# b4rtaz/distributed-llama

Hardware: NVIDIA B200
Metric: decode tokens/sec (batch-1 sequence, greedy) + prefill TTFT, Llama-3.1-8B q40 (higher is better)
Workload: dtype q40 weights, q80 activations (int8 dp4a), bf16 KV, f32 accum; 1 GPU; model=llama-3.1-8b, global_batch=1, seq_len=84, prompt_len=64, parallelism=tp1, l2_policy=weights per step (4.22 GB/GPU) >> 126 MB L2, no flush needed

## Files before the change

csrc/cuda/engine.cu:

```cuda
#include <algorithm>
#include <cstdlib>
#include <cstring>
#include <vector>

#include "engine_api.h"
#include "kernels.h"

namespace dl {

uint32_t gHiddenAct = 0;

static_assert(kApiMaxRanks == kMaxRanks, "engine_api.h and kernels.h disagree on the rank limit");

struct Buffers {
    int *tokens, *pos;
    float *x, *qkv, *z, *h, *logits;
    float *attnPartial;
    unsigned int *attnCounters;
    int *history;
    int *expertIdx;
    float *expertWeight;
    float *routerLogits;
    unsigned int *routerCounter;
    float *moeScratch;
    unsigned int *moeCounters;
    int *pTokens, *pPos;
    float *px, *pqkv;
    void *pxn, *pzb, *phb;
    float *pAttnPartial;
    unsigned int *pAttnCounters;
    float *argVal;
    int *argIdx;
    unsigned int *argCounter;
};

struct Engine {
    EngineConfig cfg{};
    CommPtrs comm{};
    bool tp = false;
    std::vector<LayerPtrs> layers;
    GlobalPtrs g{};
    Buffers b{};
    std::vector<void *> kCache, vCache;
    std::vector<void *> owned;
    cudaGraphExec_t decodeGraph = nullptr;
    cudaStream_t captureStream = nullptr;
    int lastError = 0;
    uint64_t *trace = nullptr;
    uint32_t traceCap = 0;
    bool traceAllCtas = false;
    MegaLayer *megaLayers = nullptr;
    unsigned int *megaCounter = nullptr;
    uint2 *megaX2 = nullptr;
    uint32_t megaFlags = 0;
    uint2 *megaX = nullptr, *megaQkv = nullptr, *megaZ = nullptr, *megaH = nullptr;
    unsigned int *megaSeq = nullptr;
    unsigned int *abortHost = nullptr, *abortDev = nullptr;
    uint32_t megaInflight = 2;
    uint32_t megaCtas = 0;
    bool useMega = false;
    bool lastDecodeMega = false, megaFallbackWarned = false;
    unsigned long long *rngState = nullptr;
    float *probScratch = nullptr;
    unsigned int *gatherEpoch = nullptr, *gatherBlockCounter = nullptr;
    float **gatherUcDev = nullptr;
    unsigned int **flagUcDev = nullptr;
    uint32_t vocabLimit = 0;
    bool prefillFusedAr = false;
    bool tcAttn = true;
    bool fusedAttn = true, fusedArgmax = true, useTma = true;
};

#define DL_TRY(expr)                    \
    do {                                \
        const int _r = (expr);          \
        if (_r != 0) return _r;         \
    } while (0)

static EmbTable embTable(const Engine &e) {
    EmbTable t{};
    t.rowsPerRank = e.g.embRowsPerRank;
    if (t.rowsPerRank == 0) t.shard[0] = e.g.embedding;
    else for (int r = 0; r < kMaxRanks; r++) t.shard[r] = e.g.embeddingPeers[r];
    return t;
}

constexpr uint32_t kArenaMaxCtas = 256;

static EngineConfig applyLimits(EngineConfig c) {
    if (c.nExperts > 0) c.maxBatch = 1;
    if (c.maxPrefill > 256) c.maxPrefill = 256;
    return c;
}

struct ArenaLayout {
    uint64_t slotsOff, flagsOff, candValOff, gatherOff, prefillSlotsOff, bytes;
};

static ArenaLayout arenaLayout(const EngineConfig &c) {
    auto align = [](uint64_t x) { return (x + 255) / 256 * 256; };
    ArenaLayout a{};
    uint64_t off = 0;
    a.slotsOff = off; off = align(off + 2ull * c.nRanks * c.maxBatch * c.dim * 8);
    a.flagsOff = off; off = align(off + 2ull * c.nRanks * kArenaMaxCtas * 4);
    a.candValOff = off; off = align(off + kMaxRanks * 8);
    a.gatherOff = off; off = align(off + (uint64_t)c.maxBatch * c.vocabFull * 4);
    a.prefillSlotsOff = off; off = align(off + 2ull * c.nRanks * c.maxPrefill * c.dim * 8);
    a.bytes = off;
    return a;
}

static void fillAr(const Engine &e, ArArgs &ar, uint32_t parity) {
    const EngineConfig &c = e.cfg;
    const ArenaLayout L = arenaLayout(c);
    ar.nRanks = c.nRanks; ar.rank = c.rank; ar.parity = parity; ar.maxCtas = kArenaMaxCtas; ar.slotStride = c.maxBatch * c.dim; ar.dim = c.dim;
    ar.slotsMc = e.comm.mcArena ? (uint64_t *)((uint8_t *)e.comm.mcArena + L.slotsOff) : nullptr;
    for (uint32_t r = 0; r < c.nRanks && r < (uint32_t)kMaxRanks; r++) {
        uint8_t *base = (uint8_t *)e.comm.arena[r];
        ar.slots[r] = (uint64_t *)(base + L.slotsOff);
        ar.cand[r] = (uint64_t *)(base + L.candValOff);
    }
}

static uint32_t localVocabLimit(const Engine &e) {
    return (e.vocabLimit && e.vocabLimit < e.cfg.vocab) ? e.vocabLimit : e.cfg.vocab;
}

static int gemvSel(const Engine &e, int pro, int epi, int nb, const GemvArgs &a, int numSms, cudaStream_t stream, bool pdl) {
    if (e.cfg.wType != 0) return gemvDense((int)e.cfg.wType, pro, epi, nb, a, numSms, stream, pdl);
    if (a.ar.nRanks > 1) {
        const int r = gemvQ40Tma(pro, epi, nb, a, numSms, stream, pdl);
        return r == 1 ? -30 : r;
    }
    return e.useTma ? gemvQ40Auto(pro, epi, nb, a, numSms, stream, pdl) : gemvQ40(pro, epi, nb, a, numSms, stream, pdl);
}

static int runMoe(Engine &e, const LayerPtrs &L, float *out, bool fusedAr, uint64_t *trace13, uint64_t *trace2, cudaStream_t stream,
                  bool pdl) {
    const EngineConfig &c = e.cfg;
    if (c.wType != 0) return -34;
    RouterArgs ro{};
    ro.x = e.b.x; ro.normW = L.norm1; ro.gate = L.moeGate; ro.eps = c.eps; ro.dim = c.dim; ro.nExperts = c.nExperts;
    ro.k = c.nActiveExperts; ro.logits = e.b.routerLogits; ro.counter = e.b.routerCounter; ro.expertIdx = e.b.expertIdx;
    ro.expertWeight = e.b.expertWeight;
    DL_TRY(launchMoeRouter(ro, 1, stream, pdl));
    const uint32_t perSlot = c.numSms / c.nActiveExperts > 0 ? c.numSms / c.nActiveExperts : 1;
    GemvArgs a{};
    a.qs = (const uint32_t *)L.w13Qs; a.scales = (const __half *)L.w13Sc; a.d = 2 * c.ffDim; a.n = c.dim;
    a.in = e.b.x; a.inStride = c.dim; a.normW = L.norm1; a.eps = c.eps; a.out = e.b.h; a.outStride = c.ffDim; a.trace = trace13;
    a.moeCtasPerSlot = perSlot; a.kActive = c.nActiveExperts; a.expertIdx = e.b.expertIdx; a.outSlotStride = c.ffDim;
    a.expertQsStride = (uint64_t)2 * c.ffDim * (c.dim / 8); a.expertScaleStride = (uint64_t)2 * c.ffDim * (c.dim / 32);
    a.moeFirstExpert = c.moeFirstExpert; a.moeNumLocal = c.moeNumLocal;
    { const int r = gemvQ40Tma(PRO_RMSNORM_, EPI_SWIGLU_, 1, a, c.numSms, stream, pdl); if (r != 0) return r == 1 ? -31 : r; }
    a = GemvArgs{};
    a.qs = (const uint32_t *)L.w2Qs; a.scales = (const __half *)L.w2Sc; a.d = c.dim; a.n = c.ffDim;
    a.in = e.b.h; a.inStride = c.ffDim; a.inSlotStride = c.ffDim; a.out = out; a.outStride = c.dim; a.trace = trace2;
    a.moeCtasPerSlot = perSlot; a.kActive = c.nActiveExperts; a.expertIdx = e.b.expertIdx; a.expertWeight = e.b.expertWeight;
    a.expertQsStride = (uint64_t)c.dim * (c.ffDim / 8); a.expertScaleStride = (uint64_t)c.dim * (c.ffDim / 32);
    a.moeFirstExpert = c.moeFirstExpert; a.moeNumLocal = c.moeNumLocal; a.moeScratch = e.b.moeScratch; a.moeCounters = e.b.moeCounters;
    if (fusedAr) fillAr(e, a.ar, 1);
    { const int r = gemvQ40Tma(PRO_PLAIN_, EPI_MOE_DOWN_, 1, a, c.numSms, stream, pdl); if (r != 0) return r == 1 ? -32 : r; }
    return 0;
}

static int engineDecodeMega(Engine &e, bool greedyAdvance, cudaStream_t stream) {
    const EngineConfig &c = e.cfg;
    if (!e.megaLayers || c.nExperts > 0 || c.wType != 0) return 1;
    MegaArgs m{};
    m.layers = e.megaLayers; m.nLayers = c.nLayers; m.dim = c.dim; m.nHeads = c.nHeads; m.nKvHeads = c.nKvHeads; m.headDim = c.headDim;
    m.ffDim = c.ffDim; m.vocab = c.vocab; m.vocabFull = c.vocabFull; m.seqLen = c.seqLen; m.nSplits = c.nSplits; m.eps = c.eps;
    m.embedding = embTable(e); m.finalNorm = e.g.finalNorm; m.rope = e.g.rope;
    m.wclsQs = (const uint8_t *)e.g.wclsQs; m.wclsSc = (const uint8_t *)e.g.wclsSc;
    m.tokens = e.b.tokens; m.pos = e.b.pos; m.history = e.b.history;
    m.logits = e.b.logits; m.maxInflight = e.megaInflight;
    m.xW = e.megaX; m.xW2 = e.megaX2; m.flags = e.megaFlags; m.qkvW = e.megaQkv; m.zW = e.megaZ; m.hF = (float *)e.megaH; m.launchSeq = e.megaSeq; m.abortFlag = e.abortDev;
    m.syncNs = (e.tp && e.megaSeq) ? (unsigned long long *)(e.megaSeq + 2) : nullptr;
    m.attnPartial = e.b.attnPartial; m.attnCounters = e.b.attnCounters;
    m.argVal = e.b.argVal; m.argIdx = e.b.argIdx; m.argCounter = e.b.argCounter; m.gridCounter = e.megaCounter;
    m.rowOffsetGlobal = c.rank * c.vocab; m.greedyAdvance = greedyAdvance ? 1u : 0u; m.vocabLimit = e.vocabLimit;
    m.trace = e.trace;
    m.traceCtas = e.traceAllCtas ? c.numSms : 1u;
    m.traceStride = e.traceAllCtas ? (uint32_t)(((size_t)e.traceCap * 4) / c.numSms) : 0u;
    if (e.tp) fillAr(e, m.ar, 0);
    return launchMegaDecode(m, (int)(e.megaCtas ? e.megaCtas : c.numSms), stream);
}

static int engineForward(Engine &e, int nb, int logitsMode, bool greedyAdvance, cudaStream_t stream) {
    const EngineConfig &c = e.cfg;
    const bool pdl = c.usePdl != 0;
    const uint32_t qDim = c.nHeads * c.headDim, kvDim = c.nKvHeads * c.headDim, qkvDim = qDim + 2 * kvDim;
    if (nb < 1 || (uint32_t)nb > c.maxBatch || (nb & (nb - 1))) return -10;
    e.lastDecodeMega = false;
    if (nb == 1 && logitsMode == 1 && e.useMega) {
        const int r = engineDecodeMega(e, greedyAdvance, stream);
        if (r != 1) { e.lastDecodeMega = r == 0; return r; }
        if (!e.megaFallbackWarned) {
            std::fprintf(stderr, "dl_engine: the persistent decode kernel cannot run this configuration (shape, shared memory or co-residency); "
                                 "using the multi-kernel path\n");
            e.megaFallbackWarned = true;
        }
    }
    uint32_t slot = 0;
    auto nextTrace = [&]() -> uint64_t * { uint64_t *t = (e.trace && slot < e.traceCap) ? e.trace + (size_t)slot * 4 : nullptr; slot++; return t; };

    DL_TRY(launchEmbedding(embTable(e), e.b.tokens, e.b.x, c.dim, c.dim, c.vocabFull, nb, stream));
    for (uint32_t l = 0; l < c.nLayers; l++) {
        const LayerPtrs &L = e.layers[l];
        GemvArgs a{};
        a.qs = (const uint32_t *)L.qkvQs; a.scales = (const __half *)L.qkvSc; a.d = qkvDim; a.n = c.dim;
        a.in = e.b.x; a.inStride = c.dim; a.normW = L.norm0; a.eps = c.eps; a.out = e.b.qkv; a.outStride = qkvDim; a.trace = nextTrace();
        DL_TRY(gemvSel(e, PRO_RMSNORM_, EPI_STORE_, nb, a, c.numSms, stream, pdl));
        if (nb == 1 && e.fusedAttn) {
            AttnFusedArgs f{};
            f.qkv = e.b.qkv; f.pos = e.b.pos; f.rope = e.g.rope; f.qNorm = L.qNorm; f.kNorm = L.kNorm; f.eps = c.eps;
            f.kCache = (__nv_bfloat16 *)e.kCache[l]; f.vCache = (__nv_bfloat16 *)e.vCache[l];
            f.nHeads = c.nHeads; f.nKvHeads = c.nKvHeads; f.headDim = c.headDim; f.seqLen = c.seqLen; f.nSplits = c.nSplits;
            f.partial = e.b.attnPartial; f.counters = e.b.attnCounters; f.out = e.b.z; f.trace = nextTrace();
            DL_TRY(launchAttnFused(f, stream, pdl));
        } else {
            RopeKvArgs r{};
            r.qkv = e.b.qkv; r.qkvStride = qkvDim; r.pos = e.b.pos; r.rope = e.g.rope; r.qNorm = L.qNorm; r.kNorm = L.kNorm;
            r.eps = c.eps; r.nHeads = c.nHeads; r.nKvHeads = c.nKvHeads; r.headDim = c.headDim; r.seqLen = c.seqLen;
            r.kCache = (__nv_bfloat16 *)e.kCache[l]; r.vCache = (__nv_bfloat16 *)e.vCache[l];
            DL_TRY(launchRopeKv(r, nb, stream, pdl));
            AttnArgs t{};
            t.qkv = e.b.qkv; t.qkvStride = qkvDim; t.pos = e.b.pos; t.kCache = r.kCache; t.vCache = r.vCache;
            t.nHeads = c.nHeads; t.nKvHeads = c.nKvHeads; t.headDim = c.headDim; t.seqLen = c.seqLen; t.nSplits = c.nSplits;
            t.partial = e.b.attnPartial; t.counters = e.b.attnCounters; t.out = e.b.z; t.outStride = qDim;
            DL_TRY(launchAttnDecode(t, nb, stream, pdl));
        }
        a = GemvArgs{};
        a.qs = (const uint32_t *)L.woQs; a.scales = (const __half *)L.woSc; a.d = c.dim; a.n = qDim;
        a.in = e.b.z; a.inStride = qDim; a.out = e.b.x; a.outStride = c.dim; a.trace = nextTrace();
        if (e.tp) fillAr(e, a.ar, 0);
        DL_TRY(gemvSel(e, PRO_PLAIN_, EPI_RESIDUAL_, nb, a, c.numSms, stream, pdl));
        if (c.nExperts > 0) {
            if (nb != 1) return -13;
            nextTrace();
            uint64_t *t13 = nextTrace(), *t2 = nextTrace();
            DL_TRY(runMoe(e, L, e.b.x, e.tp, t13, t2, stream, pdl));
            continue;
        }
        a = GemvArgs{};
        a.qs = (const uint32_t *)L.w13Qs; a.scales = (const __half *)L.w13Sc; a.d = 2 * c.ffDim; a.n = c.dim;
        a.in = e.b.x; a.inStride = c.dim; a.normW = L.norm1; a.eps = c.eps; a.out = e.b.h; a.outStride = c.ffDim; a.trace = nextTrace();
        DL_TRY(gemvSel(e, PRO_RMSNORM_, EPI_SWIGLU_, nb, a, c.numSms, stream, pdl));
        a = GemvArgs{};
        a.qs = (const uint32_t *)L.w2Qs; a.scales = (const __half *)L.w2Sc; a.d = c.dim; a.n = c.ffDim;
        a.in = e.b.h; a.inStride = c.ffDim; a.out = e.b.x; a.outStride = c.dim; a.trace = nextTrace();
        if (e.tp) fillAr(e, a.ar, 1);
        DL_TRY(gemvSel(e, PRO_PLAIN_, EPI_RESIDUAL_, nb, a, c.numSms, stream, pdl));
    }
    if (logitsMode != 0) {
        GemvArgs a{};
        a.qs = (const uint32_t *)e.g.wclsQs; a.scales = (const __half *)e.g.wclsSc; a.d = c.vocab; a.n = c.dim;
        a.normW = e.g.finalNorm; a.eps = c.eps; a.inStride = c.dim; a.outStride = c.vocab; a.out = e.b.logits; a.trace = nextTrace();
        if (logitsMode == 1) {
            a.in = e.b.x + (size_t)(nb - 1) * c.dim;
            int r = 1;
            if (greedyAdvance && e.fusedArgmax && c.wType == 0) {
                a.argVal = e.b.argVal; a.argIdx = e.b.argIdx; a.argCounter = e.b.argCounter;
                a.tokenOut = e.b.tokens; a.posInOut = e.b.pos; a.history = e.b.history; a.historyCap = c.seqLen;
                a.rowOffsetGlobal = c.rank * c.vocab; a.vocabLimit = e.vocabLimit;
                if (e.tp) fillAr(e, a.ar, 0);
                r = gemvQ40Tma(PRO_RMSNORM_, EPI_ARGMAX_, 1, a, c.numSms, stream, pdl);
                if (r < 0) return r;
            }
            if (r == 1) {
                if (greedyAdvance && e.tp) return -33;
                a.argVal = nullptr; a.argIdx = nullptr; a.argCounter = nullptr; a.tokenOut = nullptr; a.posInOut = nullptr; a.history = nullptr;
                a.ar = ArArgs{};
                DL_TRY(gemvSel(e, PRO_RMSNORM_, EPI_STORE_, 1, a, c.numSms, stream, pdl));
                if (greedyAdvance)
                    DL_TRY(launchArgmaxAdvance(e.b.logits, localVocabLimit(e), e.b.tokens, e.b.pos, e.b.history, c.seqLen, stream, pdl));
            }
        } else {
            a.in = e.b.x;
            DL_TRY(gemvSel(e, PRO_RMSNORM_, EPI_STORE_, nb, a, c.numSms, stream, pdl));
            if (greedyAdvance) {
                if (e.tp) return -33;
                DL_TRY(launchArgmaxAdvance(e.b.logits, localVocabLimit(e), e.b.tokens, e.b.pos, e.b.history, c.seqLen, stream, pdl));
            }
        }
    }
    return 0;
}

static int enginePrefill(Engine &e, uint32_t T, uint32_t p0, int wantLogits, cudaStream_t stream) {
    const EngineConfig &c = e.cfg;
    const GlobalPtrs &g = e.g;
    const Buffers &b = e.b;
    const bool pdl = c.usePdl != 0;
    const uint32_t qDim = c.nHeads * c.headDim, kvDim = c.nKvHeads * c.headDim, qkvDim = qDim + 2 * kvDim;
    if (T < 1 || T > c.maxPrefill) return -11;
    if (c.wType != 0) return -35;
    const bool tp = e.tp;
    ArArgs arP{};
    if (tp) {
        fillAr(e, arP, 0);
        const uint64_t off = arenaLayout(c).prefillSlotsOff;
        arP.slotStride = c.maxPrefill * c.dim;
        for (uint32_t r = 0; r < c.nRanks; r++) arP.slots[r] = (uint64_t *)((uint8_t *)e.comm.arena[r] + off);
        arP.slotsMc = e.comm.mcArena ? (uint64_t *)((uint8_t *)e.comm.mcArena + off) : nullptr;
    }
    DL_TRY(launchEmbedding(embTable(e), b.pTokens, b.px, c.dim, c.dim, c.vocabFull, (int)T, stream));
    for (uint32_t l = 0; l < c.nLayers; l++) {
        const LayerPtrs &L = e.layers[l];
        DL_TRY(launchRmsNormBf16(b.px, c.dim, L.norm0, b.pxn, c.dim, c.dim, c.eps, T, stream, pdl));
        DL_TRY(gemmQ40Tc(GEPI_STORE_F32_, L.qkvQs, L.qkvSc, qkvDim, c.dim, b.pxn, c.dim, T, b.pqkv, qkvDim, c.numSms, stream, pdl));
        RopeKvArgs r{};
        r.qkv = b.pqkv; r.qkvStride = qkvDim; r.pos = b.pPos; r.rope = g.rope; r.qNorm = L.qNorm; r.kNorm = L.kNorm;
        r.eps = c.eps; r.nHeads = c.nHeads; r.nKvHeads = c.nKvHeads; r.headDim = c.headDim; r.seqLen = c.seqLen;
        r.kCache = (__nv_bfloat16 *)e.kCache[l]; r.vCache = (__nv_bfloat16 *)e.vCache[l];
        DL_TRY(launchRopeKv(r, (int)T, stream, pdl));
        int attnRc = 1;
        if (e.tcAttn) {
            AttnPrefillArgs ap{};
            ap.qkv = b.pqkv; ap.qkvStride = qkvDim; ap.T = T; ap.p0 = p0; ap.nHeads = c.nHeads; ap.nKvHeads = c.nKvHeads;
            ap.headDim = c.headDim; ap.seqLen = c.seqLen; ap.kCache = r.kCache; ap.vCache = r.vCache;
            ap.out = (__nv_bfloat16 *)b.pzb; ap.outStride = qDim;
            attnRc = launchAttnPrefillTc(ap, stream, pdl);
            if (attnRc < 0) return attnRc;
        }
        if (attnRc == 1) {
            AttnArgs t{};
            t.qkv = b.pqkv; t.qkvStride = qkvDim; t.pos = b.pPos; t.kCache = r.kCache; t.vCache = r.vCache;
            t.nHeads = c.nHeads; t.nKvHeads = c.nKvHeads; t.headDim = c.headDim; t.seqLen = c.seqLen; t.nSplits = 1;
            t.partial = b.pAttnPartial; t.counters = b.pAttnCounters; t.out = nullptr; t.outStride = qDim; t.outBf16 = (__nv_bfloat16 *)b.pzb;
            DL_TRY(launchAttnDecode(t, (int)T, stream, pdl));
        }
        if (tp && !e.prefillFusedAr) {
            arP.parity = 0;
            DL_TRY(gemmQ40Tc(GEPI_STORE_F32_, L.woQs, L.woSc, c.dim, qDim, b.pzb, qDim, T, b.pqkv, c.dim, c.numSms, stream, pdl));
            DL_TRY(launchArResidual(b.px, b.pqkv, c.dim, T, arP, stream, pdl));
        } else if (tp) { arP.parity = 0; DL_TRY(gemmQ40TcAr(L.woQs, L.woSc, c.dim, qDim, b.pzb, qDim, T, b.px, c.dim, c.numSms, stream, arP)); }
        else DL_TRY(gemmQ40Tc(GEPI_RESIDUAL_, L.woQs, L.woSc, c.dim, qDim, b.pzb, qDim, T, b.px, c.dim, c.numSms, stream, pdl));
        if (c.nExperts > 0) {
            MoePrefillArgs mo{};
            mo.x = b.px; mo.xnScratch = b.pxn; mo.norm = L.norm1; mo.gate = L.moeGate; mo.w13Qs = L.w13Qs; mo.w13Sc = L.w13Sc;
            mo.w2Qs = L.w2Qs; mo.w2Sc = L.w2Sc; mo.T = T; mo.dim = c.dim; mo.ff = c.ffDim; mo.nExperts = c.nExperts; mo.k = c.nActiveExperts;
            mo.firstLocal = c.moeFirstExpert; mo.nLocal = c.moeNumLocal; mo.eps = c.eps; mo.numSms = (int)c.numSms;
            if (tp) { arP.parity = 1; mo.ar = arP; }
            const int mr = moePrefillFfn(mo, stream);
            if (mr != 0) return mr == 1 ? -36 : mr;
            continue;
        }
        DL_TRY(launchRmsNormBf16(b.px, c.dim, L.norm1, b.pxn, c.dim, c.dim, c.eps, T, stream, pdl));
        DL_TRY(gemmQ40Tc(GEPI_SWIGLU_BF16_, L.w13Qs, L.w13Sc, 2 * c.ffDim, c.dim, b.pxn, c.dim, T, b.phb, c.ffDim, c.numSms, stream, pdl));
        if (tp && !e.prefillFusedAr) {
            arP.parity = 1;
            DL_TRY(gemmQ40Tc(GEPI_STORE_F32_, L.w2Qs, L.w2Sc, c.dim, c.ffDim, b.phb, c.ffDim, T, b.pqkv, c.dim, c.numSms, stream, pdl));
            DL_TRY(launchArResidual(b.px, b.pqkv, c.dim, T, arP, stream, pdl));
        } else if (tp) { arP.parity = 1; DL_TRY(gemmQ40TcAr(L.w2Qs, L.w2Sc, c.dim, c.ffDim, b.phb, c.ffDim, T, b.px, c.dim, c.numSms, stream, arP)); }
        else DL_TRY(gemmQ40Tc(GEPI_RESIDUAL_, L.w2Qs, L.w2Sc, c.dim, c.ffDim, b.phb, c.ffDim, T, b.px, c.dim, c.numSms, stream, pdl));
    }
    if (wantLogits) {
        GemvArgs a{};
        a.qs = (const uint32_t *)g.wclsQs; a.scales = (const __half *)g.wclsSc; a.d = c.vocab; a.n = c.dim;
        a.normW = g.finalNorm; a.eps = c.eps; a.inStride = c.dim; a.outStride = c.vocab; a.out = b.logits;
        a.in = b.px + (size_t)(T - 1) * c.dim;
        DL_TRY(gemvSel(e, PRO_RMSNORM_, EPI_STORE_, 1, a, c.numSms, stream, false));
    }
    return 0;
}

static bool allocBuffers(Engine &e) {
    const EngineConfig &c = e.cfg;
    bool ok = true;
    auto zeroed = [&](size_t bytes) -> void * {
        void *p = nullptr;
        if (!ok || bytes == 0) return nullptr;
        if (cudaMalloc(&p, bytes) != cudaSuccess) { ok = false; return nullptr; }
        e.owned.push_back(p);
        ok = cudaMemset(p, 0, bytes) == cudaSuccess;
        return p;
    };
    const size_t mb = c.maxBatch, mp = c.maxPrefill, dim = c.dim, ff = c.ffDim, heads = c.nHeads, hd = c.headDim;
    const size_t kAct = std::max(1u, c.nActiveExperts), qDim = heads * hd, qkvDim = qDim + 2 * (size_t)c.nKvHeads * hd;
    Buffers &b = e.b;
    b.tokens = (int *)zeroed(mb * 4); b.pos = (int *)zeroed(mb * 4);
    b.x = (float *)zeroed(mb * dim * 4); b.qkv = (float *)zeroed(mb * qkvDim * 4); b.z = (float *)zeroed(mb * qDim * 4);
    b.h = (float *)zeroed(std::max(mb, kAct) * ff * 4); b.logits = (float *)zeroed(mb * c.vocab * 4);
    b.attnPartial = (float *)zeroed(mb * heads * c.nSplits * (hd + 2) * 4); b.attnCounters = (unsigned int *)zeroed(mb * heads * 4);
    b.history = (int *)zeroed(((size_t)c.seqLen + 1) * 4);
    b.expertIdx = (int *)zeroed(mb * kAct * 4); b.expertWeight = (float *)zeroed(mb * kAct * 4);
    b.routerLogits = (float *)zeroed(mb * std::max(1u, c.nExperts) * 4); b.routerCounter = (unsigned int *)zeroed(mb * 4);
    b.moeScratch = (float *)zeroed(kAct * dim * 4); b.moeCounters = (unsigned int *)zeroed(256 * 4);
    b.pTokens = (int *)zeroed(mp * 4); b.pPos = (int *)zeroed(mp * 4);
    b.px = (float *)zeroed(mp * dim * 4); b.pqkv = (float *)zeroed(mp * std::max(qkvDim, dim) * 4);
    b.pxn = zeroed(mp * dim * 2); b.pzb = zeroed(mp * qDim * 2); b.phb = zeroed(mp * ff * 2);
    b.pAttnPartial = (float *)zeroed(mp * heads * (hd + 2) * 4); b.pAttnCounters = (unsigned int *)zeroed(mp * heads * 4);
    b.argVal = (float *)zeroed(256 * 4); b.argIdx = (int *)zeroed(256 * 4); b.argCounter = (unsigned int *)zeroed(4 * 4);
    for (uint32_t l = 0; l < c.nLayers; l++) {
        e.kCache.push_back(zeroed((size_t)c.nKvHeads * c.seqLen * hd * 2));
        e.vCache.push_back(zeroed((size_t)c.nKvHeads * c.seqLen * hd * 2));
    }
    return ok && cudaDeviceSynchronize() == cudaSuccess;
}

}

using dl::Engine;

DL_EXPORT void *dl_engine_create(const dl::EngineConfig *cfg) {
    Engine *e = new Engine();
    e->cfg = dl::applyLimits(*cfg);
    dl::gHiddenAct = cfg->hiddenAct;
    e->layers.resize(cfg->nLayers);
    e->fusedAttn = std::getenv("DL_NO_FUSED_ATTN") == nullptr;
    e->fusedArgmax = std::getenv("DL_NO_FUSED_ARGMAX") == nullptr;
    e->useTma = std::getenv("DL_NO_TMA") == nullptr;
    e->tcAttn = std::getenv("DL_NO_TC_ATTN") == nullptr;
    e->prefillFusedAr = std::getenv("DL_PREFILL_FUSED_AR") != nullptr;
    if (e->cfg.numSms == 0) {
        int dev = 0, sms = 0;
        cudaGetDevice(&dev);
        cudaDeviceGetAttribute(&sms, cudaDevAttrMultiProcessorCount, dev);
        e->cfg.numSms = (uint32_t)sms;
    }
    if (e->cfg.nSplits == 0) e->cfg.nSplits = std::max(1u, std::min(32u, 2 * e->cfg.numSms / std::max(1u, e->cfg.nHeads)));
    if (!dl::allocBuffers(*e)) {
        dl_engine_destroy(e);
        return nullptr;
    }
    return e;
}

DL_EXPORT void dl_engine_destroy(void *h) {
    Engine *e = (Engine *)h;
    if (!e) return;
    if (e->decodeGraph) cudaGraphExecDestroy(e->decodeGraph);
    if (e->captureStream) cudaStreamDestroy(e->captureStream);
    if (e->megaLayers) cudaFree(e->megaLayers);
    if (e->megaCounter) cudaFree(e->megaCounter);
    for (void *q : {(void *)e->megaX, (void *)e->megaX2, (void *)e->megaQkv, (void *)e->megaZ, (void *)e->megaH, (void *)e->megaSeq}) if (q) cudaFree(q);
    if (e->abortHost) cudaFreeHost(e->abortHost);
    for (void *p : e->owned) cudaFree(p);
    delete e;
}

DL_EXPORT int dl_engine_set_layer(void *h, uint32_t layer, const dl::LayerPtrs *p) {
    Engine *e = (Engine *)h;
    if (layer >= e->layers.size()) return -1;
    e->layers[layer] = *p;
    return 0;
}

DL_EXPORT int dl_engine_set_globals(void *h, const dl::GlobalPtrs *p) {
    ((Engine *)h)->g = *p;
    return 0;
}

DL_EXPORT int dl_engine_get_config(void *h, dl::EngineConfig *cfg) {
    *cfg = ((Engine *)h)->cfg;
    return 0;
}

DL_EXPORT int dl_engine_buffers(void *h, dl::EngineBuffers *out) {
    const Engine *e = (Engine *)h;
    const dl::Buffers &b = e->b;
    *out = dl::EngineBuffers{b.tokens, b.pos, b.history, b.logits, b.x, b.pTokens, b.pPos, e->kCache.data(), e->vCache.data()};
    return 0;
}

DL_EXPORT size_t dl_engine_arena_bytes(const dl::EngineConfig *cfg) { return dl::arenaLayout(dl::applyLimits(*cfg)).bytes; }

DL_EXPORT int dl_engine_enable_mega(void *h, int enable) {
    Engine *e = (Engine *)h;
    if (enable && !e->megaLayers) {
        std::vector<dl::MegaLayer> tab(e->layers.size());
        for (size_t l = 0; l < tab.size(); l++) {
            const dl::LayerPtrs &L = e->layers[l];
            dl::MegaLayer &m = tab[l];
            m.qkvQs = (const uint8_t *)L.qkvQs; m.qkvSc = (const uint8_t *)L.qkvSc; m.woQs = (const uint8_t *)L.woQs; m.woSc = (const uint8_t *)L.woSc;
            m.w13Qs = (const uint8_t *)L.w13Qs; m.w13Sc = (const uint8_t *)L.w13Sc; m.w2Qs = (const uint8_t *)L.w2Qs; m.w2Sc = (const uint8_t *)L.w2Sc;
            m.norm0 = L.norm0; m.norm1 = L.norm1; m.qNorm = L.qNorm; m.kNorm = L.kNorm;
            m.kCache = (__nv_bfloat16 *)e->kCache[l]; m.vCache = (__nv_bfloat16 *)e->vCache[l];
        }
        DL_CUDA_CHECK(cudaMalloc(&e->megaLayers, tab.size() * sizeof(dl::MegaLayer)));
        DL_CUDA_CHECK(cudaMemcpy(e->megaLayers, tab.data(), tab.size() * sizeof(dl::MegaLayer), cudaMemcpyHostToDevice));
        DL_CUDA_CHECK(cudaMalloc(&e->megaCounter, 256));
        DL_CUDA_CHECK(cudaMemset(e->megaCounter, 0, 256));
        const dl::EngineConfig &c = e->cfg;
        const size_t qDim = (size_t)c.nHeads * c.headDim, qkvDim = qDim + 2 * (size_t)c.nKvHeads * c.headDim;
        auto allocW = [](uint2 **p, size_t n) {
            const size_t bytes = (n + 8) * sizeof(uint2);
            if (cudaMalloc(p, bytes) != cudaSuccess) return false;
            return cudaMemset(*p, 0, bytes) == cudaSuccess;
        };
        if (!allocW(&e->megaX, c.dim) || !allocW(&e->megaX2, c.dim) || !allocW(&e->megaQkv, qkvDim) || !allocW(&e->megaZ, qDim) || !allocW(&e->megaH, c.ffDim)) return -41;
        DL_CUDA_CHECK(cudaMalloc(&e->megaSeq, 256));
        const unsigned int one = 1;
        DL_CUDA_CHECK(cudaMemset(e->megaSeq, 0, 256));
        DL_CUDA_CHECK(cudaMemcpy(e->megaSeq, &one, sizeof(one), cudaMemcpyHostToDevice));
        if (!e->abortHost) {
            DL_CUDA_CHECK(cudaHostAlloc((void **)&e->abortHost, 64, cudaHostAllocMapped));
            std::memset(e->abortHost, 0, 64);
            DL_CUDA_CHECK(cudaHostGetDevicePointer((void **)&e->abortDev, e->abortHost, 0));
        }
        if (const char *g = std::getenv("DL_MEGA_CTAS")) e->megaCtas = (uint32_t)std::atoi(g);
        if (const char *g = std::getenv("DL_MEGA_FLAGS")) e->megaFlags = (uint32_t)std::atoi(g);
        if (const char *g = std::getenv("DL_MEGA_INFLIGHT")) e->megaInflight = (uint32_t)std::atoi(g);
    }
    e->useMega = enable != 0;
    return 0;
}

DL_EXPORT int dl_engine_set_vocab_limit(void *h, uint32_t limit) {
    Engine *e = (Engine *)h;
    if (e->vocabLimit != limit && e->decodeGraph) { cudaGraphExecDestroy(e->decodeGraph); e->decodeGraph = nullptr; }
    e->vocabLimit = limit;
    return 0;
}

DL_EXPORT unsigned long long dl_engine_sync_ns(void *h) {
    Engine *e = (Engine *)h;
    unsigned long long v = 0;
    if (e->megaSeq && cudaMemcpy(&v, e->megaSeq + 2, sizeof(v), cudaMemcpyDeviceToHost) != cudaSuccess) return 0ull;
    return v;
}

DL_EXPORT int dl_engine_aborted(void *h) {
    Engine *e = (Engine *)h;
    return (e->abortHost && *e->abortHost) ? 1 : 0;
}

DL_EXPORT int dl_engine_sampler_seed(void *h, unsigned long long seed) {
    Engine *e = (Engine *)h;
    const dl::EngineConfig &c = e->cfg;
    if (!e->rngState) {
        DL_CUDA_CHECK(cudaMalloc(&e->rngState, 64));
        DL_CUDA_CHECK(cudaMalloc(&e->probScratch, ((size_t)c.vocab * (c.nRanks ? c.nRanks : 1) + 16) * sizeof(float)));
        DL_CUDA_CHECK(cudaMalloc(&e->gatherEpoch, 64));
        DL_CUDA_CHECK(cudaMemset(e->gatherEpoch, 0, 64));
        DL_CUDA_CHECK(cudaMalloc(&e->gatherBlockCounter, 64));
        DL_CUDA_CHECK(cudaMemset(e->gatherBlockCounter, 0, 64));
        if (e->tp) {
            const dl::ArenaLayout L = dl::arenaLayout(c);
            float *g[dl::kApiMaxRanks] = {};
            unsigned int *f[dl::kApiMaxRanks] = {};
            for (uint32_t r = 0; r < c.nRanks; r++) {
                g[r] = (float *)((uint8_t *)e->comm.arena[r] + L.gatherOff);
                f[r] = (unsigned int *)((uint8_t *)e->comm.arena[r] + L.flagsOff);
            }
            DL_CUDA_CHECK(cudaMalloc(&e->gatherUcDev, sizeof(g)));
            DL_CUDA_CHECK(cudaMalloc(&e->flagUcDev, sizeof(f)));
            DL_CUDA_CHECK(cudaMemcpy(e->gatherUcDev, g, sizeof(g), cudaMemcpyHostToDevice));
            DL_CUDA_CHECK(cudaMemcpy(e->flagUcDev, f, sizeof(f), cudaMemcpyHostToDevice));
        }
    }
    if (seed == 0) seed = 0x9E3779B97F4A7C15ull;
    DL_CUDA_CHECK(cudaMemcpy(e->rngState, &seed, sizeof(seed), cudaMemcpyHostToDevice));
    return 0;
}

DL_EXPORT int dl_engine_sample(void *h, float temperature, float topp, cudaStream_t stream) {
    Engine *e = (Engine *)h;
    const dl::EngineConfig &c = e->cfg;
    if (!e->rngState) return -50;
    const uint32_t nR = e->tp ? c.nRanks : 1;
    const uint32_t full = c.vocab * nR;
    const uint32_t n = (e->vocabLimit && e->vocabLimit < full) ? e->vocabLimit : full;
    if (nR == 1)
        return dl::launchSample(e->b.logits, e->probScratch, n, temperature, topp, e->rngState, e->b.tokens, e->b.pos, e->b.history, c.seqLen,
                                nullptr, nullptr, 1, stream);
    const dl::ArenaLayout L = dl::arenaLayout(c);
    uint8_t *mine = (uint8_t *)e->comm.arena[c.rank];
    float *gatherLocal = (float *)(mine + L.gatherOff);
    unsigned int *flagLocal = (unsigned int *)(mine + L.flagsOff);
    float *gatherMc = e->comm.mcArena ? (float *)((uint8_t *)e->comm.mcArena + L.gatherOff) : nullptr;
    unsigned int *flagMc = e->comm.mcArena ? (unsigned int *)((uint8_t *)e->comm.mcArena + L.flagsOff) : nullptr;
    DL_TRY(dl::launchLogitsGather(e->b.logits, c.vocab, c.rank, nR, gatherMc, e->gatherUcDev, flagMc, e->flagUcDev, e->gatherBlockCounter, stream));
    return dl::launchSample(gatherLocal, e->probScratch, n, temperature, topp, e->rngState, e->b.tokens, e->b.pos, e->b.history, c.seqLen, flagLocal,
                            e->gatherEpoch, nR, stream);
}

DL_EXPORT int dl_engine_set_comm(void *h, const dl::CommPtrs *p) {
    Engine *e = (Engine *)h;
    e->comm = *p;
    e->tp = e->cfg.nRanks > 1;
    return 0;
}

DL_EXPORT int dl_engine_set_trace(void *h, uint64_t *buf, uint32_t capLaunches) {
    ((Engine *)h)->trace = buf;
    ((Engine *)h)->traceCap = capLaunches;
    return 0;
}

DL_EXPORT int dl_engine_set_trace_all(void *h, int allCtas) {
    ((Engine *)h)->traceAllCtas = allCtas != 0;
    return 0;
}

DL_EXPORT int dl_engine_mega_active(void *h) { return ((Engine *)h)->lastDecodeMega ? 1 : 0; }

DL_EXPORT int dl_engine_forward(void *h, int nb, int logitsMode, int greedyAdvance, cudaStream_t stream) {
    return dl::engineForward(*(Engine *)h, nb, logitsMode, greedyAdvance != 0, stream);
}

DL_EXPORT int dl_engine_forward_part(void *h, int nb, uint32_t layer, int part, float *ybuf, cudaStream_t stream) {
    Engine &e = *(Engine *)h;
    const dl::EngineConfig &c = e.cfg;
    const uint32_t qDim = c.nHeads * c.headDim, kvDim = c.nKvHeads * c.headDim, qkvDim = qDim + 2 * kvDim;
    if (nb < 1 || (uint32_t)nb > c.maxBatch || (nb & (nb - 1))) return -10;
    if (part == 0) return dl::launchEmbedding(embTable(e), e.b.tokens, e.b.x, c.dim, c.dim, c.vocabFull, nb, stream);
    if (part == 3 || part == 4) {
        dl::GemvArgs a{};
        a.qs = (const uint32_t *)e.g.wclsQs; a.scales = (const __half *)e.g.wclsSc; a.d = c.vocab; a.n = c.dim;
        a.normW = e.g.finalNorm; a.eps = c.eps; a.inStride = c.dim; a.outStride = c.vocab; a.out = e.b.logits;
        a.in = part == 3 ? e.b.x + (size_t)(nb - 1) * c.dim : e.b.x;
        return dl::gemvSel(e, dl::PRO_RMSNORM_, dl::EPI_STORE_, part == 3 ? 1 : nb, a, c.numSms, stream, false);
    }
    if (layer >= c.nLayers) return -1;
    const dl::LayerPtrs &L = e.layers[layer];
    dl::GemvArgs a{};
    if (part == 1) {
        a.qs = (const uint32_t *)L.qkvQs; a.scales = (const __half *)L.qkvSc; a.d = qkvDim; a.n = c.dim;
        a.in = e.b.x; a.inStride = c.dim; a.normW = L.norm0; a.eps = c.eps; a.out = e.b.qkv; a.outStride = qkvDim;
        DL_TRY(dl::gemvSel(e, dl::PRO_RMSNORM_, dl::EPI_STORE_, nb, a, c.numSms, stream, false));
        dl::RopeKvArgs r{};
        r.qkv = e.b.qkv; r.qkvStride = qkvDim; r.pos = e.b.pos; r.rope = e.g.rope; r.qNorm = L.qNorm; r.kNorm = L.kNorm;
        r.eps = c.eps; r.nHeads = c.nHeads; r.nKvHeads = c.nKvHeads; r.headDim = c.headDim; r.seqLen = c.seqLen;
        r.kCache = (__nv_bfloat16 *)e.kCache[layer]; r.vCache = (__nv_bfloat16 *)e.vCache[layer];
        DL_TRY(dl::launchRopeKv(r, nb, stream, false));
        dl::AttnArgs t{};
        t.qkv = e.b.qkv; t.qkvStride = qkvDim; t.pos = e.b.pos; t.kCache = r.kCache; t.vCache = r.vCache;
        t.nHeads = c.nHeads; t.nKvHeads = c.nKvHeads; t.headDim = c.headDim; t.seqLen = c.seqLen; t.nSplits = c.nSplits;
        t.partial = e.b.attnPartial; t.counters = e.b.attnCounters; t.out = e.b.z; t.outStride = qDim;
        DL_TRY(dl::launchAttnDecode(t, nb, stream, false));
        a = dl::GemvArgs{};
        a.qs = (const uint32_t *)L.woQs; a.scales = (const __half *)L.woSc; a.d = c.dim; a.n = qDim;
        a.in = e.b.z; a.inStride = qDim; a.out = ybuf; a.outStride = c.dim;
        return dl::gemvSel(e, dl::PRO_PLAIN_, dl::EPI_STORE_, nb, a, c.numSms, stream, false);
    }
    if (part == 2 && c.nExperts > 0) {
        if (nb != 1) return -13;
        DL_CUDA_CHECK(cudaMemsetAsync(ybuf, 0, (size_t)c.dim * sizeof(float), stream));
        return dl::runMoe(e, L, ybuf, false, nullptr, nullptr, stream, false);
    }
    if (part == 2) {
        a.qs = (const uint32_t *)L.w13Qs; a.scales = (const __half *)L.w13Sc; a.d = 2 * c.ffDim; a.n = c.dim;
        a.in = e.b.x; a.inStride = c.dim; a.normW = L.norm1; a.eps = c.eps; a.out = e.b.h; a.outStride = c.ffDim;
        DL_TRY(dl::gemvSel(e, dl::PRO_RMSNORM_, dl::EPI_SWIGLU_, nb, a, c.numSms, stream, false));
        a = dl::GemvArgs{};
        a.qs = (const uint32_t *)L.w2Qs; a.scales = (const __half *)L.w2Sc; a.d = c.dim; a.n = c.ffDim;
        a.in = e.b.h; a.inStride = c.ffDim; a.out = ybuf; a.outStride = c.dim;
        return dl::gemvSel(e, dl::PRO_PLAIN_, dl::EPI_STORE_, nb, a, c.numSms, stream, false);
    }
    return -2;
}

DL_EXPORT int dl_engine_prefill(void *h, uint32_t T, uint32_t p0, int wantLogits, cudaStream_t stream) {
    return dl::enginePrefill(*(Engine *)h, T, p0, wantLogits, stream);
}

DL_EXPORT int dl_engine_capture_decode(void *h) {
    Engine *e = (Engine *)h;
    if (!e->captureStream) DL_CUDA_CHECK(cudaStreamCreateWithFlags(&e->captureStream, cudaStreamNonBlocking));
    if (e->decodeGraph) { cudaGraphExecDestroy(e->decodeGraph); e->decodeGraph = nullptr; }
    DL_CUDA_CHECK(cudaStreamBeginCapture(e->captureStream, cudaStreamCaptureModeThreadLocal));
    const int r = dl::engineForward(*e, 1, 1, true, e->captureStream);
    cudaGraph_t graph = nullptr;
    const cudaError_t endErr = cudaStreamEndCapture(e->captureStream, &graph);
    if (r != 0) { if (graph) cudaGraphDestroy(graph); return r; }
    DL_CUDA_CHECK(endErr);
    DL_CUDA_CHECK(cudaGraphInstantiate(&e->decodeGraph, graph, 0));
    cudaGraphDestroy(graph);
    return 0;
}

DL_EXPORT int dl_engine_decode_graph(void *h, int nSteps, cudaStream_t stream) {
    Engine *e = (Engine *)h;
    if (!e->decodeGraph) return -20;
    for (int i = 0; i < nSteps; i++) DL_CUDA_CHECK(cudaGraphLaunch(e->decodeGraph, stream));
    return 0;
}
```

csrc/cuda/kernels.h:

```cpp
#pragma once
#include "common.cuh"

namespace dl {

enum { PRO_RMSNORM_ = 0, PRO_PLAIN_ = 1 };
enum { EPI_STORE_ = 0, EPI_RESIDUAL_ = 1, EPI_SWIGLU_ = 2, EPI_ARGMAX_ = 3, EPI_MOE_DOWN_ = 4 };

constexpr int kMaxRanks = 8;
extern uint32_t gHiddenAct;

struct ArArgs {
    uint32_t nRanks, rank, parity, maxCtas;
    uint32_t slotStride;
    uint32_t dim;
    uint64_t *slots[kMaxRanks];
    uint64_t *cand[kMaxRanks];
    uint64_t *slotsMc;
};

struct GemvArgs {
    const uint32_t *qs;
    const __half *scales;
    uint32_t d, n;
    const float *in;
    const float *normW;
    float eps;
    float *out;
    uint32_t inStride, outStride;
    uint32_t maxTileRows;
    const int *expertIdx;
    uint32_t slot, kActive;
    uint64_t expertQsStride, expertScaleStride;
    const float *expertWeight;
    float *argVal;
    int *argIdx;
    unsigned int *argCounter;
    int *tokenOut, *posInOut, *history;
    uint32_t historyCap;
    uint32_t rowOffsetGlobal;
    uint64_t *trace;
    uint32_t moeCtasPerSlot, moeFirstExpert, moeNumLocal;
    uint32_t inSlotStride, outSlotStride;
    float *moeScratch;
    unsigned int *moeCounters;
    ArArgs ar;
    uint32_t act;
    uint32_t vocabLimit;
};
int gemvQ40(int pro, int epi, int nb, GemvArgs a, int numSms, cudaStream_t stream, bool pdl);
int gemvQ40Tma(int pro, int epi, int nb, GemvArgs a, int numSms, cudaStream_t stream, bool pdl);
inline int gemvQ40Auto(int pro, int epi, int nb, const GemvArgs &a, int numSms, cudaStream_t stream, bool pdl) {
    const int r = gemvQ40Tma(pro, epi, nb, a, numSms, stream, pdl);
    return r == 1 ? gemvQ40(pro, epi, nb, a, numSms, stream, pdl) : r;
}

int gemvDense(int wtype, int pro, int epi, int nb, GemvArgs a, int numSms, cudaStream_t stream, bool pdl);

struct RopeKvArgs {
    float *qkv;
    uint32_t qkvStride;
    const int *pos;
    const float *rope;
    const float *qNorm;
    const float *kNorm;
    float eps;
    uint32_t nHeads, nKvHeads, headDim, seqLen;
    __nv_bfloat16 *kCache;
    __nv_bfloat16 *vCache;
};
int launchRopeKv(const RopeKvArgs &a, int nb, cudaStream_t stream, bool pdl);

struct AttnArgs {
    const float *qkv;
    uint32_t qkvStride;
    const int *pos;
    const __nv_bfloat16 *kCache, *vCache;
    uint32_t nHeads, nKvHeads, headDim, seqLen, nSplits;
    float *partial;
    unsigned int *counters;
    float *out;
    uint32_t outStride;
    __nv_bfloat16 *outBf16;
};
int launchAttnDecode(const AttnArgs &a, int nb, cudaStream_t stream, bool pdl);

struct AttnPrefillArgs {
    const float *qkv;
    uint32_t qkvStride;
    uint32_t T, p0;
    uint32_t nHeads, nKvHeads, headDim, seqLen;
    const __nv_bfloat16 *kCache, *vCache;
    __nv_bfloat16 *out;
    uint32_t outStride;
};
int launchAttnPrefillTc(const AttnPrefillArgs &a, cudaStream_t stream, bool pdl = false);

struct AttnFusedArgs {
    const float *qkv;
    const int *pos;
    const float *rope;
    const float *qNorm, *kNorm;
    float eps;
    __nv_bfloat16 *kCache, *vCache;
    uint32_t nHeads, nKvHeads, headDim, seqLen, nSplits;
    float *partial;
    unsigned int *counters;
    float *out;
    uint64_t *trace;
};
int launchAttnFused(const AttnFusedArgs &a, cudaStream_t stream, bool pdl);

struct RouterArgs {
    const float *x;
    const float *normW;
    const float *gate;
    float eps;
    uint32_t dim, nExperts, k;
    float *logits;
    unsigned int *counter;
    int *expertIdx;
    float *expertWeight;
};
int launchMoeRouter(const RouterArgs &a, int nb, cudaStream_t stream, bool pdl);

struct EmbTable {
    const float *shard[kMaxRanks];
    uint32_t rowsPerRank;
    __host__ __device__ const float *row(uint32_t tok, uint32_t dim) const {
        if (rowsPerRank == 0) return shard[0] + (size_t)tok * dim;
        const uint32_t r = tok / rowsPerRank;
        return shard[r] + (size_t)(tok - r * rowsPerRank) * dim;
    }
};
int launchEmbedding(const EmbTable &table, const int *tokens, float *x, uint32_t dim, uint32_t xStride, uint32_t vocab, int nb,
                    cudaStream_t stream);
int launchArgmaxAdvance(const float *logits, uint32_t vocab, int *tokenOut, int *pos, int *history, uint32_t historyCap,
                        cudaStream_t stream, bool pdl);

int launchSample(const float *logits, float *probs, uint32_t n, float temperature, float topp, unsigned long long *rng, int *tokenOut, int *pos,
                 int *history, uint32_t historyCap, const unsigned int *gatherFlag, unsigned int *gatherEpoch, uint32_t nRanks,
                 cudaStream_t stream);
int launchLogitsGather(const float *local, uint32_t v0, uint32_t rank, uint32_t nRanks, float *gatherMc, float *const *gatherUcDev,
                       unsigned int *flagMc, unsigned int *const *flagUcDev, unsigned int *blockCounter, cudaStream_t stream);

struct MegaLayer {
    const uint8_t *qkvQs, *qkvSc, *woQs, *woSc, *w13Qs, *w13Sc, *w2Qs, *w2Sc;
    const float *norm0, *norm1, *qNorm, *kNorm;
    __nv_bfloat16 *kCache, *vCache;
};

struct MegaPhase {
    uint32_t d, n, nblk, nseg;
    uint32_t stageRows;
    uint32_t pairsQ, pairsRem;
    uint32_t recipNseg, gInc, segInc, rotInc;
};

struct MegaArgs {
    const MegaLayer *layers;
    uint32_t nLayers, dim, nHeads, nKvHeads, headDim, ffDim, vocab, vocabFull, seqLen, nSplits;
    float eps;
    EmbTable embedding;
    const float *finalNorm, *rope;
    const uint8_t *wclsQs, *wclsSc;
    int *tokens, *pos, *history;
    float *logits;
    uint2 *xW2;
    uint32_t flags;
    uint2 *xW, *qkvW, *zW;
    float *hF;
    unsigned int *launchSeq;
    unsigned int *abortFlag;
    unsigned long long *syncNs;
    float *attnPartial;
    unsigned int *attnCounters;
    float *argVal;
    int *argIdx;
    unsigned int *argCounter;
    unsigned int *gridCounter;
    uint32_t stageBytes, nStages, planeBlocks, partialFloats;
    uint32_t maxInflight;
    MegaPhase ph[5];
    uint32_t rowOffsetGlobal;
    uint32_t greedyAdvance;
    uint32_t act, vocabLimit;
    uint64_t *trace;
    uint32_t traceCtas, traceStride;
    ArArgs ar;
};

int launchMegaDecode(MegaArgs m, int numSms, cudaStream_t stream);

enum { GEPI_STORE_F32_ = 0, GEPI_RESIDUAL_ = 1, GEPI_SWIGLU_BF16_ = 2, GEPI_STORE_BF16_ = 3 };
int gemmQ40Tc(int epi, const void *qs, const void *scales, uint32_t d, uint32_t n, const void *act, uint32_t actStride, uint32_t T,
              void *out, uint32_t outStride, int numSms, cudaStream_t stream, bool pdl);
int gemmQ40TcAr(const void *qs, const void *scales, uint32_t d, uint32_t n, const void *act, uint32_t actStride, uint32_t T, void *out,
                uint32_t outStride, int numSms, cudaStream_t stream, const ArArgs &ar);
int gemmQ40TcGrouped(int epi, const void *qs, const void *scales, uint32_t nGroups, uint32_t grpRows, uint32_t n, const void *act,
                     uint32_t actStride, uint32_t rowsTotal, uint32_t maxTokens, const int *grpCount, const int *grpOffset, void *out,
                     uint32_t outStride, int numSms, cudaStream_t stream);
struct MoePrefillArgs {
    float *x;
    void *xnScratch;
    const float *norm, *gate;
    const void *w13Qs, *w13Sc, *w2Qs, *w2Sc;
    uint32_t T, dim, ff, nExperts, k, firstLocal, nLocal;
    float eps;
    int numSms;
    ArArgs ar;
};
int moePrefillFfn(const MoePrefillArgs &a, cudaStream_t stream);
template <typename... KArgs, typename... Args>
inline cudaError_t launchPdl(void (*kernel)(KArgs...), dim3 grid, dim3 block, size_t smem, cudaStream_t stream, bool pdl, Args... args) {
    cudaLaunchConfig_t cfg{};
    cfg.gridDim = grid; cfg.blockDim = block; cfg.dynamicSmemBytes = smem; cfg.stream = stream;
    cudaLaunchAttribute attr[1];
    attr[0].id = cudaLaunchAttributeProgrammaticStreamSerialization;
    attr[0].val.programmaticStreamSerializationAllowed = pdl ? 1 : 0;
    cfg.attrs = attr; cfg.numAttrs = 1;
    return cudaLaunchKernelEx(&cfg, kernel, KArgs(args)...);
}

int launchArResidual(float *x, const float *partial, uint32_t dim, uint32_t T, const ArArgs &ar, cudaStream_t stream, bool pdl = false);
int launchRmsNormBf16(const float *x, uint32_t xStride, const float *w, void *y, uint32_t yStride, uint32_t n, float eps, uint32_t T,
                      cudaStream_t stream, bool pdl = false);

}
```

csrc/cuda/mega_decode.cu:

```cuda
#include <type_traits>

#include "kernels.h"
#include "tma_common.cuh"

namespace dl {

enum { MP_QKV = 0, MP_WO = 1, MP_W13 = 2, MP_W2 = 3, MP_LOGITS = 4 };

static uint32_t megaStageRows(uint32_t n, uint32_t stageBytes) {
    const uint32_t rowBytes = (n / 32) * 18;
    uint32_t sr = stageBytes / rowBytes;
    sr = sr / 4 * 4;
    return sr > 64 ? 64 : sr;
}

struct MegaSmem {
    uint8_t *ring;
    uint4 *planeA, *planeB;
    float *dxs, *dx8, *partial, *red, *rope;
    uint64_t *fullBar, *emptyBar;
};

constexpr uint32_t kSpinCheck = 1u << 12;
constexpr uint32_t kSpinLimit = 1u << 27;

struct SpinGuard {
    volatile unsigned int *abortFlag;
    uint32_t n = 0;
    __device__ __forceinline__ explicit SpinGuard(unsigned int *f) : abortFlag(f) {}
    __device__ __forceinline__ bool tick() {
        if ((++n & (kSpinCheck - 1)) != 0) return false;
        if (abortFlag && *abortFlag) return true;
        if (n >= kSpinLimit) {
            if (abortFlag) *abortFlag = 1u;
            return true;
        }
        return false;
    }
};

__device__ __forceinline__ void gridBarrier(unsigned int *ctr, unsigned int &target, int tid, unsigned int *abortFlag) {
    consumerBarrier();
    if (tid == 0) {
        asm volatile("red.relaxed.gpu.global.add.u32 [%0], 1;" ::"l"(ctr) : "memory");
        target += gridDim.x;
        unsigned int v;
        SpinGuard g(abortFlag);
        do {
            asm volatile("ld.relaxed.gpu.global.u32 %0, [%1];" : "=r"(v) : "l"(ctr) : "memory");
        } while (v < target && !g.tick());
    }
    consumerBarrier();
}

__device__ __forceinline__ void gridBarrierFenced(unsigned int *ctr, unsigned int &target, int tid, unsigned int *abortFlag) {
    consumerBarrier();
    if (tid == 0) {
        asm volatile("red.release.gpu.global.add.u32 [%0], 1;" ::"l"(ctr) : "memory");
        target += gridDim.x;
        unsigned int v;
        SpinGuard g(abortFlag);
        do {
            asm volatile("ld.acquire.gpu.global.u32 %0, [%1];" : "=r"(v) : "l"(ctr) : "memory");
        } while (v < target && !g.tick());
    }
    consumerBarrier();
}

__device__ __forceinline__ void stW(uint2 *p, float v, uint32_t epoch) {
    asm volatile("st.relaxed.gpu.global.v2.u32 [%0], {%1, %2};" ::"l"(p), "r"(__float_as_uint(v)), "r"(epoch) : "memory");
}
__device__ __forceinline__ uint4 ldW2(const uint2 *p) {
    uint4 v;
    asm volatile("ld.relaxed.gpu.global.v4.u32 {%0, %1, %2, %3}, [%4];" : "=r"(v.x), "=r"(v.y), "=r"(v.z), "=r"(v.w) : "l"(p) : "memory");
    return v;
}
__device__ __forceinline__ uint2 ldW(const uint2 *p) {
    uint2 v;
    asm volatile("ld.relaxed.gpu.global.v2.u32 {%0, %1}, [%2];" : "=r"(v.x), "=r"(v.y) : "l"(p) : "memory");
    return v;
}
__device__ __forceinline__ float ldWwait(const uint2 *p, uint32_t epoch, unsigned int *abortFlag) {
    uint2 v = ldW(p);
    if (v.y != epoch) {
        SpinGuard g(abortFlag);
        do { __nanosleep(100); v = ldW(p); } while (v.y != epoch && !g.tick());
    }
    return __uint_as_float(v.x);
}
__device__ __forceinline__ float4 ldW4wait(const uint2 *base, uint32_t i4, uint32_t epoch, unsigned int *abortFlag) {
    const uint2 *p = base + (size_t)i4 * 4;
    uint4 a = ldW2(p), b = ldW2(p + 2);
    if (a.y != epoch || a.w != epoch || b.y != epoch || b.w != epoch) {
        SpinGuard g(abortFlag);
        do { __nanosleep(100); a = ldW2(p); b = ldW2(p + 2); } while ((a.y != epoch || a.w != epoch || b.y != epoch || b.w != epoch) && !g.tick());
    }
    return make_float4(__uint_as_float(a.x), __uint_as_float(a.z), __uint_as_float(b.x), __uint_as_float(b.z));
}

struct RingPos {
    uint32_t st, par;
    __device__ __forceinline__ void advance(uint32_t nStages) {
        if (++st == nStages) { st = 0; par ^= 1u; }
    }
};

__device__ __forceinline__ void megaTile(const MegaPhase &P, uint32_t &pairBegin, uint32_t &tileRows) {
    const uint32_t b = blockIdx.x;
    pairBegin = b * P.pairsQ + min(b, P.pairsRem);
    tileRows = 2 * (P.pairsQ + (b < P.pairsRem ? 1u : 0u));
}

template <int PRO, int EPI, bool IN_PLAIN = false>
__device__ void megaGemv(const MegaArgs &m, const MegaSmem &sm, const MegaPhase &P, const uint2 *in, uint32_t inEpoch, const float *normW,
                         uint2 *outW, uint32_t outEpoch, float *outF, uint32_t arParity, RingPos &ring, int tid, uint32_t &slot,
                         const float *inF = nullptr, const uint2 *resW = nullptr) {
    auto stamp = [&]() { if (m.trace && tid == 0 && blockIdx.x < m.traceCtas) m.trace[(size_t)blockIdx.x * m.traceStride + slot] = globalTimerNs(); slot++; };
    const int lane = tid & 31, warp = tid >> 5;
    const uint32_t n = P.n;
    const uint32_t nblk = P.nblk, nseg = P.nseg;
    const uint32_t rowQsBytes = nblk * 16;
    uint32_t pairBegin, tileRows;
    megaTile(P, pairBegin, tileRows);
    const uint32_t rowBase = pairBegin * 2;
    const uint32_t SR = P.stageRows;
    uint4 *planeA = sm.planeA, *planeB = sm.planeB;
    float *dxs = sm.dxs, *dx8 = sm.dx8, *partial = sm.partial, *red = sm.red;

    float resid = 0.f;
    if (EPI == EPI_RESIDUAL_ && (uint32_t)tid < tileRows) resid = __uint_as_float(ldW((resW ? resW : outW) + rowBase + tid).x);

    {
        const uint32_t nVec = n / 4;
        constexpr int kMaxVec = PRO == PRO_RMSNORM_ ? 4 : 8;
        constexpr uint32_t kChunkVec = kMaxVec * kConsumerThreads;
        uint8_t *pa = reinterpret_cast<uint8_t *>(planeA);
        uint8_t *pb = reinterpret_cast<uint8_t *>(planeB);
        for (uint32_t vecBase = 0; vecBase < nVec; vecBase += kChunkVec) {
            float4 xv[kMaxVec];
            float4 wv[PRO == PRO_RMSNORM_ ? kMaxVec : 1];
            if (PRO == PRO_RMSNORM_) {
#pragma unroll
                for (int k = 0; k < kMaxVec; k++) {
                    const uint32_t i = vecBase + k * kConsumerThreads + tid;
                    wv[k] = i < nVec ? __ldg(reinterpret_cast<const float4 *>(normW) + i) : make_float4(0.f, 0.f, 0.f, 0.f);
                }
            }
            float ss = 0.f;
#pragma unroll
            for (int k = 0; k < kMaxVec; k++) {
                const uint32_t i = vecBase + k * kConsumerThreads + tid;
                if (IN_PLAIN) xv[k] = i < nVec ? __ldcg(reinterpret_cast<const float4 *>(inF) + i) : make_float4(0.f, 0.f, 0.f, 0.f);
                else xv[k] = i < nVec ? ldW4wait(in, i, inEpoch, m.abortFlag) : make_float4(0.f, 0.f, 0.f, 0.f);
                ss += xv[k].x * xv[k].x + xv[k].y * xv[k].y + xv[k].z * xv[k].z + xv[k].w * xv[k].w;
            }
            float inv = 1.f;
            if (PRO == PRO_RMSNORM_) {
                ss = consumerSum(ss, red);
                inv = rsqrtf(ss / (float)n + m.eps);
            }
#pragma unroll
            for (int k = 0; k < kMaxVec; k++) {
                const uint32_t i = vecBase + k * kConsumerThreads + tid;
                if (vecBase + k * kConsumerThreads >= nVec) break;
                const bool act = i < nVec;
                float4 v = xv[k];
                if (PRO == PRO_RMSNORM_ && act) {
                    const float4 w = wv[PRO == PRO_RMSNORM_ ? k : 0];
                    v.x = w.x * (v.x * inv); v.y = w.y * (v.y * inv); v.z = w.z * (v.z * inv); v.w = w.w * (v.w * inv);
                }
                float amax = fmaxf(fmaxf(fabsf(v.x), fabsf(v.y)), fmaxf(fabsf(v.z), fabsf(v.w)));
                amax = fmaxf(amax, __shfl_xor_sync(0xffffffffu, amax, 1));
                amax = fmaxf(amax, __shfl_xor_sync(0xffffffffu, amax, 2));
                amax = fmaxf(amax, __shfl_xor_sync(0xffffffffu, amax, 4));
                const float dq = amax / 127.f;
                const float id = dq != 0.f ? 1.f / dq : 0.f;
                const int q0 = __float2int_rn(v.x * id), q1 = __float2int_rn(v.y * id);
                const int q2 = __float2int_rn(v.z * id), q3 = __float2int_rn(v.w * id);
                int qsum = q0 + q1 + q2 + q3;
                qsum += __shfl_xor_sync(0xffffffffu, qsum, 1);
                qsum += __shfl_xor_sync(0xffffffffu, qsum, 2);
                qsum += __shfl_xor_sync(0xffffffffu, qsum, 4);
                if (act) {
                    const uint32_t b = i >> 3, sub = i & 7, kk = sub >> 1, odd = sub & 1;
                    uint8_t *wa = pa + (size_t)b * 16 + kk * 4 + odd;
                    uint8_t *wb = pb + (size_t)b * 16 + kk * 4 + odd;
                    wa[0] = (uint8_t)(int8_t)q0; wa[2] = (uint8_t)(int8_t)q1;
                    wb[0] = (uint8_t)(int8_t)q2; wb[2] = (uint8_t)(int8_t)q3;
                    if (sub == 0) {
                        const float dr = __half2float(__float2half_rn(dq));
                        dxs[b] = dr;
                        dx8[b] = dr * 8.f * (float)qsum;
                    }
                }
            }
        }
    }
    consumerBarrier();
    stamp();

    const uint32_t gInc = P.gInc, segInc = P.segInc;
    uint32_t rot = 0;
    for (uint32_t r0 = 0; r0 < tileRows; r0 += SR) {
        const uint32_t st = ring.st;
        const uint32_t rows = min(SR, tileRows - r0);
        const uint32_t nSteps = ((rows + kRowsPerStep - 1) / kRowsPerStep) * nseg;
        const uint8_t *stage = sm.ring + st * m.stageBytes;
        const uint4 *sq = reinterpret_cast<const uint4 *>(stage);
        const uint16_t *ss = reinterpret_cast<const uint16_t *>(stage + SR * rowQsBytes);
        const uint32_t firstStep = ((uint32_t)warp - rot) & (kConsumerWarps - 1);
        rot = (rot + P.rotInc) & (kConsumerWarps - 1);
        uint32_t g = (firstStep * P.recipNseg) >> 16, seg = firstStep - g * nseg;
        mbarWait(&sm.fullBar[st], ring.par);
        auto stepDot = [&](uint32_t g_, uint32_t seg_, float (&acc)[kRowsPerStep]) {
            const uint32_t blk = seg_ * 32 + lane;
            const uint32_t rl = g_ * kRowsPerStep;
#pragma unroll
            for (int r = 0; r < kRowsPerStep; r++) acc[r] = 0.f;
            if (blk < nblk) {
                const uint4 A = planeA[blk], B = planeB[blk];
                const float dxv = dxs[blk], dx8v = dx8[blk];
                const uint4 *qp = sq + rl * nblk + blk;
                const uint16_t *sp = ss + rl * nblk + blk;
#pragma unroll
                for (int r = 0; r < kRowsPerStep; r++) {
                    const uint4 q = qp[r * nblk];
                    const float dw = __half2float(__ushort_as_half(sp[r * nblk]));
                    const uint32_t ml = 0x0f0f0f0fu, mh = 0xf0f0f0f0u;
                    int lo = dp4a(q.x & ml, A.x, 0), hi = dp4a(q.x & mh, B.x, 0);
                    lo = dp4a(q.y & ml, A.y, lo); hi = dp4a(q.y & mh, B.y, hi);
                    lo = dp4a(q.z & ml, A.z, lo); hi = dp4a(q.z & mh, B.z, hi);
                    lo = dp4a(q.w & ml, A.w, lo); hi = dp4a(q.w & mh, B.w, hi);
                    acc[r] = dw * (dxv * (float)(lo + (hi >> 4)) - dx8v);
                }
            }
        };
        auto stepStore = [&](uint32_t g_, uint32_t seg_, float v) {
            const uint32_t rl = g_ * kRowsPerStep;
            if ((lane & 7) == 0) {
                const uint32_t r = lane >> 3;
                if (rl + r < rows) partial[(r0 + rl + r) * nseg + seg_] = v;
            }
        };
        auto advance = [&](uint32_t &g_, uint32_t &seg_) {
            g_ += gInc;
            seg_ += segInc;
            if (seg_ >= nseg) { seg_ -= nseg; g_++; }
        };
        uint32_t s = firstStep;
        for (; s + kConsumerWarps < nSteps; s += 2 * kConsumerWarps) {
            uint32_t g2 = g, seg2 = seg;
            advance(g2, seg2);
            float a0[kRowsPerStep], a1[kRowsPerStep];
            stepDot(g, seg, a0);
            stepDot(g2, seg2, a1);
            const float v0 = reduce4(a0[0], a0[1], a0[2], a0[3], lane);
            const float v1 = reduce4(a1[0], a1[1], a1[2], a1[3], lane);
            stepStore(g, seg, v0);
            stepStore(g2, seg2, v1);
            g = g2; seg = seg2;
            advance(g, seg);
        }
        if (s < nSteps) {
            float a0[kRowsPerStep];
            stepDot(g, seg, a0);
            stepStore(g, seg, reduce4(a0[0], a0[1], a0[2], a0[3], lane));
        }
        __syncwarp();
        if (lane == 0) mbarArrive(&sm.emptyBar[st]);
        ring.advance(m.nStages);
    }
    consumerBarrier();
    stamp();

    auto rowSum = [&](uint32_t r) {
        float v = 0.f;
        for (uint32_t sg = 0; sg < nseg; sg++) v += partial[r * nseg + sg];
        return v;
    };
    if (EPI == EPI_SWIGLU_) {
        for (uint32_t p = tid; p < tileRows / 2; p += kConsumerThreads) outF[pairBegin + p] = gateAct(rowSum(2 * p), m.act) * rowSum(2 * p + 1);
    } else if (EPI == EPI_STORE_) {
        for (uint32_t r = tid; r < tileRows; r += kConsumerThreads) stW(outW + rowBase + r, rowSum(r), outEpoch);
    } else if (EPI == EPI_RESIDUAL_) {
        if (m.ar.nRanks > 1) {
            const ArArgs &ar = m.ar;
            const size_t slotBase = (size_t)(arParity * ar.nRanks + ar.rank) * ar.slotStride;
            if ((uint32_t)tid < tileRows) {
                const uint32_t r = tid;
                const float v = rowSum(r);
                if (ar.slotsMc) {
                    const uint64_t word = (uint64_t)__float_as_uint(v) | (1ull << 32);
                    asm volatile("multimem.st.relaxed.sys.global.b64 [%0], %1;" ::"l"(ar.slotsMc + slotBase + rowBase + r), "l"(word) : "memory");
                } else {
#pragma unroll 1
                    for (uint32_t p = 0; p < ar.nRanks; p++) stLL(ar.slots[(ar.rank + p) % ar.nRanks] + slotBase + rowBase + r, __float_as_uint(v), 1u);
                }
                uint64_t *mine = ar.slots[ar.rank];
                float sum = 0.f;
                SpinGuard g(m.abortFlag);
                const bool timeIt = m.syncNs && blockIdx.x == 0 && tid == 0;
                const uint64_t tSync0 = timeIt ? globalTimerNs() : 0;
                for (uint32_t sr = 0; sr < ar.nRanks; sr++) {
                    uint64_t *w = mine + (size_t)(arParity * ar.nRanks + sr) * ar.slotStride + rowBase + r;
                    uint2 v2 = ldLL(w);
                    while (v2.y == 0u && !g.tick()) v2 = ldLL(w);
                    sum += __uint_as_float(v2.x);
                    stLL(w, 0u, 0u);
                }
                if (timeIt) *m.syncNs += globalTimerNs() - tSync0;
                stW(outW + rowBase + r, resid + sum, outEpoch);
            }
        } else if ((uint32_t)tid < tileRows) {
            stW(outW + rowBase + tid, resid + rowSum(tid), outEpoch);
        }
    } else {
        float best = -INFINITY;
        int bestIdx = 0x7fffffff;
        for (uint32_t r = tid; r < tileRows; r += kConsumerThreads) {
            const float v = rowSum(r);
            outF[rowBase + r] = v;
            if (EPI == EPI_ARGMAX_ && v > best && m.rowOffsetGlobal + rowBase + r < m.vocabLimit) { best = v; bestIdx = (int)(m.rowOffsetGlobal + rowBase + r); }
        }
        if (EPI == EPI_ARGMAX_) {
            auto better = [](float v, int i, float bv, int bi) { return v > bv || (v == bv && i < bi); };
#pragma unroll
            for (int o = 16; o > 0; o >>= 1) {
                const float ov = __shfl_xor_sync(0xffffffffu, best, o);
                const int oi = __shfl_xor_sync(0xffffffffu, bestIdx, o);
                if (better(ov, oi, best, bestIdx)) { best = ov; bestIdx = oi; }
            }
            float *sv = red;
            int *si = reinterpret_cast<int *>(red + 16);
            consumerBarrier();
            if (lane == 0) { sv[warp] = best; si[warp] = bestIdx; }
            consumerBarrier();
            __shared__ bool lastCta;
            if (warp == 0) {
                best = lane < kConsumerWarps ? sv[lane] : -INFINITY;
                bestIdx = lane < kConsumerWarps ? si[lane] : 0x7fffffff;
#pragma unroll
                for (int o = 16; o > 0; o >>= 1) {
                    const float ov = __shfl_xor_sync(0xffffffffu, best, o);
                    const int oi = __shfl_xor_sync(0xffffffffu, bestIdx, o);
                    if (better(ov, oi, best, bestIdx)) { best = ov; bestIdx = oi; }
                }
                if (lane == 0) {
                    m.argVal[blockIdx.x] = best;
                    m.argIdx[blockIdx.x] = bestIdx;
                    __threadfence();
                    const unsigned int prev = atomicAdd(m.argCounter, 1u);
                    lastCta = prev == gridDim.x - 1;
                    if (lastCta) *m.argCounter = 0;
                }
            }
            consumerBarrier();
            if (lastCta && warp == 0) {
                __threadfence();
                best = -INFINITY;
                bestIdx = 0x7fffffff;
                for (uint32_t i = lane; i < gridDim.x; i += 32) {
                    const float v = __ldcg(m.argVal + i);
                    const int ix = __ldcg(m.argIdx + i);
                    if (better(v, ix, best, bestIdx)) { best = v; bestIdx = ix; }
                }
#pragma unroll
                for (int o = 16; o > 0; o >>= 1) {
                    const float ov = __shfl_xor_sync(0xffffffffu, best, o);
                    const int oi = __shfl_xor_sync(0xffffffffu, bestIdx, o);
                    if (better(ov, oi, best, bestIdx)) { best = ov; bestIdx = oi; }
                }
                if (m.ar.nRanks > 1) {
                    const ArArgs &ar = m.ar;
                    if (lane < ar.nRanks) stLL(ar.cand[lane] + ar.rank, __float_as_uint(best), (uint32_t)bestIdx + 1u);
                    if (lane < ar.nRanks) {
                        uint64_t *w = ar.cand[ar.rank] + lane;
                        uint2 v = ldLL(w);
                        SpinGuard g(m.abortFlag);
                        while (v.y == 0u && !g.tick()) v = ldLL(w);
                        best = __uint_as_float(v.x);
                        bestIdx = (int)(v.y - 1u);
                        stLL(w, 0u, 0u);
                    } else {
                        best = -INFINITY;
                        bestIdx = 0x7fffffff;
                    }
#pragma unroll
                    for (int o = 16; o > 0; o >>= 1) {
                        const float ov = __shfl_xor_sync(0xffffffffu, best, o);
                        const int oi = __shfl_xor_sync(0xffffffffu, bestIdx, o);
                        if (better(ov, oi, best, bestIdx)) { best = ov; bestIdx = oi; }
                    }
                }
                if (lane == 0 && m.greedyAdvance) {
                    m.tokens[0] = bestIdx;
                    const int p = m.pos[0] + 1;
                    m.pos[0] = p;
                    if (m.history && (uint32_t)p < m.seqLen) m.history[p] = bestIdx;
                }
            }
        }
    }
}

template <int HD>
__device__ void megaAttention(const MegaArgs &m, const MegaSmem &sm, const MegaLayer &L, int p, int tid, uint32_t inEpoch, uint32_t outEpoch) {
    constexpr int DPL = HD / 32;
    const int lane = tid & 31, warp = tid >> 5;
    const uint32_t nPos = (uint32_t)p + 1;
    uint32_t eff = (nPos + 255) / 256;
    if (eff > m.nSplits) eff = m.nSplits;
    if (eff < 1) eff = 1;
    const uint32_t kvMul = m.nHeads / m.nKvHeads;
    const uint32_t qDim = m.nHeads * HD, kvDim = m.nKvHeads * HD;
    float *sAcc = sm.partial;
    float *sM = sm.partial + 16 * HD;
    float *sL = sM + 16;
    __shared__ bool sLast;
    const float2 *ropeRow = reinterpret_cast<const float2 *>(sm.rope) + lane * (DPL / 2);
    auto normRope = [&](float *v, const float *nw) {
        if (nw) {
            float ss = 0.f;
#pragma unroll
            for (int i = 0; i < DPL; i++) ss += v[i] * v[i];
            ss = warpSum(ss);
            const float inv = rsqrtf(ss / (float)HD + m.eps);
#pragma unroll
            for (int i = 0; i < DPL; i++) v[i] = nw[lane * DPL + i] * (v[i] * inv);
        }
#pragma unroll
        for (int k = 0; k < DPL / 2; k++) {
            const float2 cs = ropeRow[k];
            const float x0 = v[2 * k] * cs.x - v[2 * k + 1] * cs.y;
            const float x1 = v[2 * k] * cs.y + v[2 * k + 1] * cs.x;
            v[2 * k] = x0; v[2 * k + 1] = x1;
        }
    };
    for (uint32_t item = blockIdx.x; item < m.nHeads * eff; item += gridDim.x) {
        const uint32_t h = item / eff, split = item - h * eff;
        const uint32_t kvh = h / kvMul;
        const uint32_t chunk = (nPos + eff - 1) / eff;
        const uint32_t begin = split * chunk;
        const uint32_t end = min(begin + chunk, nPos);
        const bool ownsNew = end == nPos;
        const uint32_t cachedEnd = ownsNew ? end - 1 : end;
        __nv_bfloat16 *kHead = L.kCache + (size_t)kvh * m.seqLen * HD;
        __nv_bfloat16 *vHead = L.vCache + (size_t)kvh * m.seqLen * HD;
        const __nv_bfloat16 *kBase = kHead + lane * DPL;
        const __nv_bfloat16 *vBase = vHead + lane * DPL;
        constexpr int UN = 4;
        using RawT = typename std::conditional<DPL == 4, uint2, uint32_t>::type;
        RawT kRaw[UN], vRaw[UN];
        auto loadBatch = [&](uint32_t s0) {
#pragma unroll
            for (int u = 0; u < UN; u++) {
                const uint32_t s = s0 + u;
                if (s < cachedEnd) {
                    kRaw[u] = *reinterpret_cast<const RawT *>(kBase + (size_t)s * HD);
                    vRaw[u] = *reinterpret_cast<const RawT *>(vBase + (size_t)s * HD);
                }
            }
        };
        auto unpack = [&](const RawT &r, float (&o)[DPL]) {
            if constexpr (DPL == 4) {
                const float2 a0 = __bfloat1622float2(*reinterpret_cast<const __nv_bfloat162 *>(&r.x));
                const float2 a1 = __bfloat1622float2(*reinterpret_cast<const __nv_bfloat162 *>(&r.y));
                o[0] = a0.x; o[1] = a0.y; o[2] = a1.x; o[3] = a1.y;
            } else {
                const float2 a0 = __bfloat1622float2(*reinterpret_cast<const __nv_bfloat162 *>(&r));
                o[0] = a0.x; o[1] = a0.y;
            }
        };
        uint32_t s0 = begin + warp * UN;
        loadBatch(s0);
        const bool newRow = ownsNew && warp == 0;
        const uint2 *ksrc = m.qkvW + qDim + (size_t)kvh * HD + lane * DPL;
        const uint2 *vsrc = m.qkvW + qDim + kvDim + (size_t)kvh * HD + lane * DPL;
        float q[DPL], kn[DPL], vn[DPL];
        {
            const uint2 *src = m.qkvW + (size_t)h * HD + lane * DPL;
            if constexpr (DPL == 4) {
                uint4 ka0, ka1, va0, va1;
                if (newRow) { ka0 = ldW2(ksrc); ka1 = ldW2(ksrc + 2); va0 = ldW2(vsrc); va1 = ldW2(vsrc + 2); }
                const float4 v = ldW4wait(src, 0, inEpoch, m.abortFlag);
                q[0] = v.x; q[1] = v.y; q[2] = v.z; q[3] = v.w;
                if (newRow) {
                    if (ka0.y != inEpoch || ka0.w != inEpoch || ka1.y != inEpoch || ka1.w != inEpoch || va0.y != inEpoch || va0.w != inEpoch ||
                        va1.y != inEpoch || va1.w != inEpoch) {
                        const float4 a = ldW4wait(ksrc, 0, inEpoch, m.abortFlag), bq = ldW4wait(vsrc, 0, inEpoch, m.abortFlag);
                        kn[0] = a.x; kn[1] = a.y; kn[2] = a.z; kn[3] = a.w;
                        vn[0] = bq.x; vn[1] = bq.y; vn[2] = bq.z; vn[3] = bq.w;
                    } else {
                        kn[0] = __uint_as_float(ka0.x); kn[1] = __uint_as_float(ka0.z); kn[2] = __uint_as_float(ka1.x); kn[3] = __uint_as_float(ka1.z);
                        vn[0] = __uint_as_float(va0.x); vn[1] = __uint_as_float(va0.z); vn[2] = __uint_as_float(va1.x); vn[3] = __uint_as_float(va1.z);
                    }
                }
            } else {
#pragma unroll
                for (int i = 0; i < DPL; i++) q[i] = ldWwait(src + i, inEpoch, m.abortFlag);
                if (newRow) {
#pragma unroll
                    for (int i = 0; i < DPL; i++) { kn[i] = ldWwait(ksrc + i, inEpoch, m.abortFlag); vn[i] = ldWwait(vsrc + i, inEpoch, m.abortFlag); }
                }
            }
        }
        normRope(q, L.qNorm);
        const float scale = rsqrtf((float)HD);
#pragma unroll
        for (int i = 0; i < DPL; i++) q[i] *= scale;
        float mx = -INFINITY, l = 0.f, acc[DPL];
#pragma unroll
        for (int i = 0; i < DPL; i++) acc[i] = 0.f;
        if (newRow) {
            normRope(kn, L.kNorm);
            __nv_bfloat162 kb[DPL / 2], vb[DPL / 2];
#pragma unroll
            for (int k = 0; k < DPL / 2; k++) {
                kb[k] = __floats2bfloat162_rn(kn[2 * k], kn[2 * k + 1]);
                vb[k] = __floats2bfloat162_rn(vn[2 * k], vn[2 * k + 1]);
                const float2 kf = __bfloat1622float2(kb[k]), vf = __bfloat1622float2(vb[k]);
                kn[2 * k] = kf.x; kn[2 * k + 1] = kf.y;
                vn[2 * k] = vf.x; vn[2 * k + 1] = vf.y;
            }
            if (h % kvMul == 0) {
                __nv_bfloat162 *kd = reinterpret_cast<__nv_bfloat162 *>(kHead + (size_t)p * HD + lane * DPL);
                __nv_bfloat162 *vd = reinterpret_cast<__nv_bfloat162 *>(vHead + (size_t)p * HD + lane * DPL);
#pragma unroll
                for (int k = 0; k < DPL / 2; k++) { kd[k] = kb[k]; vd[k] = vb[k]; }
            }
            float dsum = 0.f;
#pragma unroll
            for (int i = 0; i < DPL; i++) dsum += q[i] * kn[i];
            dsum = warpSum(dsum);
            mx = dsum; l = 1.f;
#pragma unroll
            for (int i = 0; i < DPL; i++) acc[i] = vn[i];
        }
        for (; s0 < cachedEnd; s0 += kConsumerWarps * UN) {
            float kf[UN][DPL], vf[UN][DPL];
#pragma unroll
            for (int u = 0; u < UN; u++) {
                if (s0 + u < cachedEnd) { unpack(kRaw[u], kf[u]); unpack(vRaw[u], vf[u]); }
                else {
#pragma unroll
                    for (int i = 0; i < DPL; i++) { kf[u][i] = 0.f; vf[u][i] = 0.f; }
                }
            }
            const uint32_t cur = s0;
            if (s0 + kConsumerWarps * UN < cachedEnd) loadBatch(s0 + kConsumerWarps * UN);
            float sc[UN];
#pragma unroll
            for (int u = 0; u < UN; u++) {
                float dsum = 0.f;
#pragma unroll
                for (int i = 0; i < DPL; i++) dsum += q[i] * kf[u][i];
                sc[u] = warpSum(dsum);
            }
#pragma unroll
            for (int u = 0; u < UN; u++) {
                if (cur + u < cachedEnd) {
                    const float mNew = fmaxf(mx, sc[u]);
                    const float corr = __expf(mx - mNew);
                    const float pr = __expf(sc[u] - mNew);
                    l = l * corr + pr;
#pragma unroll
                    for (int i = 0; i < DPL; i++) acc[i] = acc[i] * corr + pr * vf[u][i];
                    mx = mNew;
                }
            }
        }
        consumerBarrier();
#pragma unroll
        for (int i = 0; i < DPL; i++) sAcc[warp * HD + lane * DPL + i] = acc[i];
        if (lane == 0) { sM[warp] = mx; sL[warp] = l; }
        consumerBarrier();
        float M = -INFINITY;
#pragma unroll
        for (int w = 0; w < kConsumerWarps; w++) M = fmaxf(M, sM[w]);
        float num = 0.f, Lsum = 0.f;
        if (tid < HD) {
#pragma unroll
            for (int w = 0; w < kConsumerWarps; w++) {
                const float wgt = (sM[w] == -INFINITY) ? 0.f : __expf(sM[w] - M);
                num += sAcc[w * HD + tid] * wgt;
                Lsum += sL[w] * wgt;
            }
        }
        uint2 *outRow = m.zW + (size_t)h * HD;
        if (eff == 1) {
            if (tid < HD) stW(outRow + tid, num / Lsum, outEpoch);
            continue;
        }
        float *pOut = m.attnPartial + ((size_t)h * m.nSplits + split) * (HD + 2);
        if (tid < HD) pOut[tid] = num;
        if (tid == 0) { pOut[HD] = M; pOut[HD + 1] = Lsum; }
        __threadfence();
        consumerBarrier();
        if (tid == 0) {
            const unsigned int prev = atomicAdd(&m.attnCounters[h], 1u);
            sLast = (prev == eff - 1);
            if (sLast) m.attnCounters[h] = 0;
        }
        consumerBarrier();
        if (sLast) {
            __threadfence();
            const float *pIn = m.attnPartial + (size_t)h * m.nSplits * (HD + 2);
            float gM = -INFINITY;
            for (uint32_t s = 0; s < eff; s++) gM = fmaxf(gM, __ldcg(pIn + (size_t)s * (HD + 2) + HD));
            if (tid < HD) {
                float n2 = 0.f, den = 0.f;
                for (uint32_t s = 0; s < eff; s++) {
                    const float w = __expf(__ldcg(pIn + (size_t)s * (HD + 2) + HD) - gM);
                    n2 += w * __ldcg(pIn + (size_t)s * (HD + 2) + tid);
                    den += w * __ldcg(pIn + (size_t)s * (HD + 2) + HD + 1);
                }
                stW(outRow + tid, n2 / den, outEpoch);
            }
        }
    }
}

template <int HD>
__global__ void __launch_bounds__(kTmaThreads, 1) megaDecodeKernel(const __grid_constant__ MegaArgs m) {
    extern __shared__ __align__(128) uint8_t smem[];
    const int tid = threadIdx.x, lane = tid & 31, warp = tid >> 5;
    MegaSmem sm;
    sm.ring = smem;
    sm.planeA = reinterpret_cast<uint4 *>(smem + (size_t)m.nStages * m.stageBytes);
    sm.planeB = sm.planeA + m.planeBlocks;
    sm.dxs = reinterpret_cast<float *>(sm.planeB + m.planeBlocks);
    sm.dx8 = sm.dxs + m.planeBlocks;
    sm.partial = sm.dx8 + m.planeBlocks;
    sm.red = sm.partial + m.partialFloats;
    sm.rope = sm.red + 32;
    sm.fullBar = reinterpret_cast<uint64_t *>(sm.rope + 128);
    sm.emptyBar = sm.fullBar + kMaxStages;

    if (tid == 0) {
        for (uint32_t s = 0; s < m.nStages; s++) {
            mbarInit(&sm.fullBar[s], 1);
            mbarInit(&sm.emptyBar[s], kConsumerWarps);
        }
        asm volatile("fence.mbarrier_init.release.cluster;" ::: "memory");
    }
    __syncthreads();
    const uint32_t qDim = m.nHeads * m.headDim, kvDim = m.nKvHeads * m.headDim, qkvDim = qDim + 2 * kvDim;

    if (warp == kConsumerWarps) {
        if (lane == 0) {
            const uint64_t policy = policyEvictFirst();
            RingPos pr{0u, 0u};
            bool wrapped = false;
            RingPos landed{0u, 0u};
            uint32_t nIssued = 0, nLanded = 0;
            const uint32_t maxInflight = m.maxInflight ? m.maxInflight : m.nStages;
            auto stream = [&](const uint8_t *qs, const uint8_t *sc, const MegaPhase &P) {
                const uint32_t rowQsBytes = P.nblk * 16, rowScBytes = P.nblk * 2;
                uint32_t pairBegin, tileRows;
                megaTile(P, pairBegin, tileRows);
                const uint32_t rowBase = pairBegin * 2, SR = P.stageRows;
                for (uint32_t r0 = 0; r0 < tileRows; r0 += SR) {
                    const uint32_t st = pr.st;
                    if (wrapped) mbarWait(&sm.emptyBar[st], pr.par ^ 1u);
                    while (nIssued - nLanded >= maxInflight) {
                        mbarWait(&sm.fullBar[landed.st], landed.par);
                        landed.advance(m.nStages);
                        nLanded++;
                    }
                    nIssued++;
                    const uint32_t rows = min(SR, tileRows - r0);
                    const uint32_t bq = rows * rowQsBytes, bs = rows * rowScBytes;
                    uint8_t *dst = sm.ring + st * m.stageBytes;
                    mbarExpectTx(&sm.fullBar[st], bq + bs);
                    tmaBulkLoad(dst, qs + (uint64_t)(rowBase + r0) * rowQsBytes, bq, &sm.fullBar[st], policy);
                    tmaBulkLoad(dst + SR * rowQsBytes, sc + (uint64_t)(rowBase + r0) * rowScBytes, bs, &sm.fullBar[st], policy);
                    pr.advance(m.nStages);
                    if (pr.st == 0) wrapped = true;
                }
            };
            for (uint32_t l = 0; l < m.nLayers; l++) {
                const MegaLayer &L = m.layers[l];
                stream(L.qkvQs, L.qkvSc, m.ph[MP_QKV]);
                stream(L.woQs, L.woSc, m.ph[MP_WO]);
                stream(L.w13Qs, L.w13Sc, m.ph[MP_W13]);
                stream(L.w2Qs, L.w2Sc, m.ph[MP_W2]);
            }
            stream(m.wclsQs, m.wclsSc, m.ph[MP_LOGITS]);
        }
        return;
    }

    unsigned int barTarget = 0;
    RingPos ring{0u, 0u};
    uint32_t slot = 0;
    auto stamp = [&]() { if (m.trace && tid == 0 && blockIdx.x < m.traceCtas) m.trace[(size_t)blockIdx.x * m.traceStride + slot] = globalTimerNs(); slot++; };
    stamp();
    const uint32_t seqBase = __ldcg(m.launchSeq) << 10;
    int p = m.pos[0];
    if (p < 0) p = 0;
    if ((uint32_t)p >= m.seqLen) p = m.seqLen - 1;
    if (tid < HD) sm.rope[tid] = m.rope[(size_t)p * HD + tid];
    {
        int tok = m.tokens[0];
        if (tok < 0 || (uint32_t)tok >= m.vocabFull) tok = 0;
        uint32_t pairBegin, tileRows;
        megaTile(m.ph[MP_WO], pairBegin, tileRows);
        if ((uint32_t)tid < tileRows) stW(m.xW + pairBegin * 2 + tid, m.embedding.row((uint32_t)tok, m.dim)[pairBegin * 2 + tid], seqBase);
    }
    gridBarrier(m.gridCounter, barTarget, tid, m.abortFlag);
    const bool noBar = (m.flags & 1u) != 0;
    auto llBarrier = [&]() { if (!noBar) gridBarrier(m.gridCounter, barTarget, tid, m.abortFlag); };
    uint2 *xA = m.xW, *xB = noBar ? m.xW2 : m.xW;
    auto prefetchVec = [&](const float *p) {
        for (uint32_t i = (blockIdx.x * kConsumerThreads + tid) * 32; i < m.dim; i += gridDim.x * kConsumerThreads * 32)
            asm volatile("prefetch.global.L2 [%0];" ::"l"(p + i));
    };
    for (uint32_t l = 0; l < m.nLayers; l++) {
        const MegaLayer &L = m.layers[l];
        const uint32_t e0 = seqBase + 5 * l;
        prefetchVec(L.norm1);
        prefetchVec(l + 1 < m.nLayers ? m.layers[l + 1].norm0 : m.finalNorm);
        stamp();
        megaGemv<PRO_RMSNORM_, EPI_STORE_>(m, sm, m.ph[MP_QKV], xA, e0, L.norm0, m.qkvW, e0 + 1, nullptr, 0, ring, tid, slot);
        stamp();
        llBarrier();
        stamp();
        megaAttention<HD>(m, sm, L, p, tid, e0 + 1, e0 + 2);
        stamp();
        llBarrier();
        stamp();
        megaGemv<PRO_PLAIN_, EPI_RESIDUAL_>(m, sm, m.ph[MP_WO], m.zW, e0 + 2, nullptr, xB, e0 + 3, nullptr, 0, ring, tid, slot, nullptr, xA);
        stamp();
        llBarrier();
        stamp();
        megaGemv<PRO_RMSNORM_, EPI_SWIGLU_>(m, sm, m.ph[MP_W13], xB, e0 + 3, L.norm1, nullptr, 0, m.hF, 0, ring, tid, slot);
        stamp();
        gridBarrierFenced(m.gridCounter, barTarget, tid, m.abortFlag);
        stamp();
        megaGemv<PRO_PLAIN_, EPI_RESIDUAL_, true>(m, sm, m.ph[MP_W2], nullptr, 0, nullptr, xA, e0 + 5, nullptr, 1, ring, tid, slot, m.hF, xB);
        stamp();
        llBarrier();
    }
    stamp();
    megaGemv<PRO_RMSNORM_, EPI_ARGMAX_>(m, sm, m.ph[MP_LOGITS], xA, seqBase + 5 * m.nLayers, m.finalNorm, nullptr, 0, m.logits, 0, ring, tid, slot);
    stamp();
    if (blockIdx.x == 0 && tid == 0) *m.launchSeq = __ldcg(m.launchSeq) + 1u;
}

int launchMegaDecode(MegaArgs m, int numSms, cudaStream_t stream) {
    if (m.headDim != 64 && m.headDim != 128) return 1;
    const uint32_t qDim = m.nHeads * m.headDim;
    const uint32_t ns[4] = {m.dim, qDim, m.ffDim, m.dim};
    uint32_t maxN = 0;
    for (uint32_t n : ns) {
        if (n % 128) return 1;
        if (n > maxN) maxN = n;
    }
    if (m.dim > 4 * kConsumerThreads * 4) return 1;
    if (5 * m.nLayers + 2 > 1023) return 1;
    const uint32_t grid = (uint32_t)numSms;
    m.act = gHiddenAct;
    if (m.vocabLimit == 0) m.vocabLimit = 0xffffffffu;
    const uint32_t ds[5] = {qDim + 2 * m.nKvHeads * m.headDim, m.dim, 2 * m.ffDim, m.dim, m.vocab};
    const uint32_t dn[5] = {m.dim, qDim, m.dim, m.ffDim, m.dim};
    uint32_t partial = 16 * m.headDim + 64;
    for (int i = 0; i < 5; i++) {
        if (ds[i] % 2) return 1;
        const uint32_t tile = 2 * ((ds[i] / 2 + grid - 1) / grid) + 2;
        const uint32_t nseg = (dn[i] / 32 + 31) / 32;
        if (tile * nseg > partial) partial = tile * nseg;
    }
    m.partialFloats = (partial + 3) / 4 * 4;
    m.planeBlocks = maxN / 32;
    const size_t fixedBytes = (size_t)m.planeBlocks * (16 + 16 + 4 + 4) + (size_t)m.partialFloats * 4 + 32 * 4 + 128 * 4 + 2 * kMaxStages * 8 + 256;
    const size_t budget = 226 * 1024;
    const uint32_t maxRowBytes = (maxN / 32) * 18;
    uint32_t stageBytes = 36 * 1024;
    if (maxRowBytes * 4 > stageBytes) stageBytes = (maxRowBytes * 4 + 127) / 128 * 128;
    if (fixedBytes + 2 * (size_t)stageBytes > budget) return 1;
    uint32_t stages = (uint32_t)((budget - fixedBytes) / stageBytes);
    if (stages > (uint32_t)kMaxStages) stages = kMaxStages;
    m.stageBytes = stageBytes;
    m.nStages = stages;
    for (int i = 0; i < 5; i++) {
        MegaPhase &P = m.ph[i];
        P.d = ds[i]; P.n = dn[i];
        P.nblk = dn[i] / 32;
        P.nseg = (P.nblk + 31) / 32;
        P.stageRows = megaStageRows(dn[i], stageBytes);
        P.pairsQ = (ds[i] / 2) / grid;
        P.pairsRem = (ds[i] / 2) % grid;
        P.recipNseg = 65536u / P.nseg + 1u;
        P.gInc = (uint32_t)kConsumerWarps / P.nseg;
        P.segInc = (uint32_t)kConsumerWarps - P.gInc * P.nseg;
        P.rotInc = ((P.stageRows / kRowsPerStep) * P.nseg) % (uint32_t)kConsumerWarps;
        for (uint32_t sft = 0; sft < (uint32_t)kConsumerWarps; sft++)
            if (((sft * P.recipNseg) >> 16) != sft / P.nseg) return 1;
    }
    if (2 * (m.ph[MP_WO].pairsQ + 1) > (uint32_t)kConsumerThreads) return 1;
    const size_t smemBytes = fixedBytes + (size_t)stages * stageBytes;
    const int v = m.headDim == 128 ? 1 : 0;
    int dev = 0;
    DL_CUDA_CHECK(cudaGetDevice(&dev));
    static size_t configured[16][2] = {};
    static int maxCoResident[16][2] = {};
    const void *fn = v ? (const void *)megaDecodeKernel<128> : (const void *)megaDecodeKernel<64>;
    const int d = dev & 15;
    if (smemBytes > configured[d][v]) {
        DL_CUDA_CHECK(cudaFuncSetAttribute(fn, cudaFuncAttributeMaxDynamicSharedMemorySize, (int)smemBytes));
        configured[d][v] = smemBytes;
        int perSm = 0, sms = 0;
        DL_CUDA_CHECK(cudaOccupancyMaxActiveBlocksPerMultiprocessor(&perSm, fn, kTmaThreads, smemBytes));
        DL_CUDA_CHECK(cudaDeviceGetAttribute(&sms, cudaDevAttrMultiProcessorCount, dev));
        maxCoResident[d][v] = perSm * sms;
    }
    if ((int)grid > maxCoResident[d][v]) return 1;
    DL_CUDA_CHECK(cudaMemsetAsync(m.gridCounter, 0, sizeof(unsigned int), stream));
    cudaLaunchConfig_t cfg{};
    cfg.gridDim = dim3(grid);
    cfg.blockDim = dim3(kTmaThreads);
    cfg.dynamicSmemBytes = smemBytes;
    cfg.stream = stream;
    cudaLaunchAttribute attr[1];
    attr[0].id = cudaLaunchAttributeCooperative;
    attr[0].val.cooperative = 1;
    cfg.attrs = attr;
    cfg.numAttrs = 1;
    if (v) DL_CUDA_CHECK(cudaLaunchKernelEx(&cfg, megaDecodeKernel<128>, m));
    else DL_CUDA_CHECK(cudaLaunchKernelEx(&cfg, megaDecodeKernel<64>, m));
    return 0;
}

}
```

csrc/cuda/repack.cu:

```cuda
#include "common.cuh"

namespace dl {

struct RepackArgs {
    const uint8_t *src;
    uint64_t srcRowPitch;
    uint64_t srcColByteOffset;
    uint32_t rows;
    uint32_t blocksPerRow;
    uint32_t *dstQs;
    __half *dstScales;
    uint32_t dstRowStride;
    uint32_t dstRowOffset;
    uint32_t headDim;
};

__global__ void __launch_bounds__(256) repackQ40Kernel(RepackArgs a) {
    const uint64_t total = (uint64_t)a.rows * a.blocksPerRow;
    for (uint64_t i = (uint64_t)blockIdx.x * blockDim.x + threadIdx.x; i < total; i += (uint64_t)gridDim.x * blockDim.x) {
        const uint32_t r = (uint32_t)(i / a.blocksPerRow);
        const uint32_t b = (uint32_t)(i % a.blocksPerRow);
        const uint8_t *s = a.src + (uint64_t)r * a.srcRowPitch + a.srcColByteOffset + (uint64_t)b * 18;
        uint8_t raw[18];
#pragma unroll
        for (int k = 0; k < 18; k++) raw[k] = s[k];
        uint32_t words[4];
#pragma unroll
        for (int w = 0; w < 4; w++) {
            uint32_t word = 0;
#pragma unroll
            for (int slot = 0; slot < 8; slot++) {
                const int eLocal = (slot < 4) ? (2 * slot) : (2 * (slot - 4) + 1);
                const int e = 8 * w + eLocal;
                const uint32_t nib = (e < 16) ? (raw[2 + e] & 0x0f) : (raw[2 + e - 16] >> 4);
                word |= nib << (4 * slot);
            }
            words[w] = word;
        }
        uint32_t rr = r;
        if (a.headDim) {
            const uint32_t h = r / a.headDim, j = r % a.headDim, half = a.headDim / 2;
            rr = h * a.headDim + (j < half ? 2 * j : 2 * (j - half) + 1);
        }
        const uint64_t dr = (uint64_t)rr * a.dstRowStride + a.dstRowOffset;
        uint4 *q = reinterpret_cast<uint4 *>(a.dstQs + (dr * a.blocksPerRow + b) * 4);
        *q = make_uint4(words[0], words[1], words[2], words[3]);
        const uint16_t sc = (uint16_t)raw[0] | ((uint16_t)raw[1] << 8);
        reinterpret_cast<uint16_t *>(a.dstScales)[dr * a.blocksPerRow + b] = sc;
    }
}

__global__ void __launch_bounds__(256) dequantDeviceQ40Kernel(const uint32_t *qs, const __half *scales, uint32_t rows,
                                                              uint32_t blocksPerRow, float *out) {
    const uint64_t total = (uint64_t)rows * blocksPerRow;
    for (uint64_t i = (uint64_t)blockIdx.x * blockDim.x + threadIdx.x; i < total; i += (uint64_t)gridDim.x * blockDim.x) {
        const float d = __half2float(scales[i]);
        const uint4 q = *reinterpret_cast<const uint4 *>(qs + i * 4);
        const uint32_t w[4] = {q.x, q.y, q.z, q.w};
        float *o = out + i * 32;
#pragma unroll
        for (int k = 0; k < 4; k++)
#pragma unroll
            for (int s = 0; s < 4; s++) {
                const uint32_t t = (w[k] >> (4 * s)) & 0x000f000fu;
                o[8 * k + 2 * s] = (float)((int)(t & 0xf) - 8) * d;
                o[8 * k + 2 * s + 1] = (float)((int)(t >> 16) - 8) * d;
            }
    }
}

}

DL_EXPORT int dl_repack_q40(const void *src, uint64_t srcRowPitch, uint64_t srcColByteOffset, uint32_t rows,
                            uint32_t blocksPerRow, void *dstQs, void *dstScales, uint32_t dstRowStride,
                            uint32_t dstRowOffset, uint32_t headDim, cudaStream_t stream) {
    dl::RepackArgs a{(const uint8_t *)src, srcRowPitch, srcColByteOffset, rows, blocksPerRow, (uint32_t *)dstQs,
                     (__half *)dstScales, dstRowStride, dstRowOffset, headDim};
    const uint64_t total = (uint64_t)rows * blocksPerRow;
    if (total == 0) return 0;
    const int grid = (int)((total + 255) / 256 < 148 * 16 ? (total + 255) / 256 : 148 * 16);
    dl::repackQ40Kernel<<<grid, 256, 0, stream>>>(a);
    DL_CUDA_CHECK(cudaGetLastError());
    return 0;
}

DL_EXPORT int dl_dequant_device_q40(const void *qs, const void *scales, uint32_t rows, uint32_t blocksPerRow, float *out,
                                    cudaStream_t stream) {
    const uint64_t total = (uint64_t)rows * blocksPerRow;
    if (total == 0) return 0;
    const int grid = (int)((total + 255) / 256 < 148 * 16 ? (total + 255) / 256 : 148 * 16);
    dl::dequantDeviceQ40Kernel<<<grid, 256, 0, stream>>>((const uint32_t *)qs, (const __half *)scales, rows, blocksPerRow, out);
    DL_CUDA_CHECK(cudaGetLastError());
    return 0;
}
```

Measured before the change: 827.3 tokens/s.

## Fuse FFN w13 and w2 in mega decode via block-major w2 slabs

```diff
diff --git a/csrc/cuda/engine.cu b/csrc/cuda/engine.cu
--- a/csrc/cuda/engine.cu
+++ b/csrc/cuda/engine.cu
@@ -54,6 +54,8 @@
     uint2 *megaX2 = nullptr;
     uint32_t megaFlags = 0;
     uint2 *megaX = nullptr, *megaQkv = nullptr, *megaZ = nullptr, *megaH = nullptr;
+    uint8_t *megaW2b = nullptr;
+    uint2 *megaPart = nullptr;
     unsigned int *megaSeq = nullptr;
     unsigned int *abortHost = nullptr, *abortDev = nullptr;
     uint32_t megaInflight = 2;
@@ -173,7 +175,7 @@
     m.wclsQs = (const uint8_t *)e.g.wclsQs; m.wclsSc = (const uint8_t *)e.g.wclsSc;
     m.tokens = e.b.tokens; m.pos = e.b.pos; m.history = e.b.history;
     m.logits = e.b.logits; m.maxInflight = e.megaInflight;
-    m.xW = e.megaX; m.xW2 = e.megaX2; m.flags = e.megaFlags; m.qkvW = e.megaQkv; m.zW = e.megaZ; m.hF = (float *)e.megaH; m.launchSeq = e.megaSeq; m.abortFlag = e.abortDev;
+    m.xW = e.megaX; m.xW2 = e.megaX2; m.flags = e.megaFlags; m.qkvW = e.megaQkv; m.zW = e.megaZ; m.hF = (float *)e.megaH; m.hW = e.megaH; m.ffPartW = e.megaPart; m.launchSeq = e.megaSeq; m.abortFlag = e.abortDev;
     m.syncNs = (e.tp && e.megaSeq) ? (unsigned long long *)(e.megaSeq + 2) : nullptr;
     m.attnPartial = e.b.attnPartial; m.attnCounters = e.b.attnCounters;
     m.argVal = e.b.argVal; m.argIdx = e.b.argIdx; m.argCounter = e.b.argCounter; m.gridCounter = e.megaCounter;
@@ -433,7 +435,8 @@
     if (e->captureStream) cudaStreamDestroy(e->captureStream);
     if (e->megaLayers) cudaFree(e->megaLayers);
     if (e->megaCounter) cudaFree(e->megaCounter);
-    for (void *q : {(void *)e->megaX, (void *)e->megaX2, (void *)e->megaQkv, (void *)e->megaZ, (void *)e->megaH, (void *)e->megaSeq}) if (q) cudaFree(q);
+    for (void *q : {(void *)e->megaX, (void *)e->megaX2, (void *)e->megaQkv, (void *)e->megaZ, (void *)e->megaH, (void *)e->megaSeq, (void *)e->megaW2b,
+                    (void *)e->megaPart}) if (q) cudaFree(q);
     if (e->abortHost) cudaFreeHost(e->abortHost);
     for (void *p : e->owned) cudaFree(p);
     delete e;
@@ -468,6 +471,23 @@
 DL_EXPORT int dl_engine_enable_mega(void *h, int enable) {
     Engine *e = (Engine *)h;
     if (enable && !e->megaLayers) {
+        const dl::EngineConfig &c = e->cfg;
+        if (const char *g = std::getenv("DL_MEGA_CTAS")) e->megaCtas = (uint32_t)std::atoi(g);
+        if (const char *g = std::getenv("DL_MEGA_FLAGS")) e->megaFlags = (uint32_t)std::atoi(g);
+        if (const char *g = std::getenv("DL_MEGA_INFLIGHT")) e->megaInflight = (uint32_t)std::atoi(g);
+        const uint32_t grid = e->megaCtas ? e->megaCtas : c.numSms, nbH = c.ffDim / 32;
+        const bool ffFused = c.nRanks <= 1 && c.nExperts == 0 && c.wType == 0 && nbH >= grid && (e->megaFlags & 1u) == 0;
+        const size_t w2bLayer = (size_t)c.dim * nbH * 18;
+        if (ffFused) {
+            if (cudaMalloc(&e->megaW2b, w2bLayer * e->layers.size()) != cudaSuccess) return -41;
+            if (cudaMalloc(&e->megaPart, (size_t)grid * c.dim * sizeof(uint2)) != cudaSuccess) return -41;
+            DL_CUDA_CHECK(cudaMemset(e->megaPart, 0, (size_t)grid * c.dim * sizeof(uint2)));
+            for (size_t l = 0; l < e->layers.size(); l++) {
+                uint8_t *qs = e->megaW2b + l * w2bLayer;
+                DL_TRY(dl::launchBlockMajorQ40(e->layers[l].w2Qs, e->layers[l].w2Sc, c.dim, nbH, qs, qs + (size_t)c.dim * nbH * 16, 0));
+            }
+            DL_CUDA_CHECK(cudaDeviceSynchronize());
+        }
         std::vector<dl::MegaLayer> tab(e->layers.size());
         for (size_t l = 0; l < tab.size(); l++) {
             const dl::LayerPtrs &L = e->layers[l];
@@ -476,12 +496,12 @@
             m.w13Qs = (const uint8_t *)L.w13Qs; m.w13Sc = (const uint8_t *)L.w13Sc; m.w2Qs = (const uint8_t *)L.w2Qs; m.w2Sc = (const uint8_t *)L.w2Sc;
             m.norm0 = L.norm0; m.norm1 = L.norm1; m.qNorm = L.qNorm; m.kNorm = L.kNorm;
             m.kCache = (__nv_bfloat16 *)e->kCache[l]; m.vCache = (__nv_bfloat16 *)e->vCache[l];
+            if (e->megaW2b) { m.w2bQs = e->megaW2b + l * w2bLayer; m.w2bSc = m.w2bQs + (size_t)c.dim * nbH * 16; }
         }
         DL_CUDA_CHECK(cudaMalloc(&e->megaLayers, tab.size() * sizeof(dl::MegaLayer)));
         DL_CUDA_CHECK(cudaMemcpy(e->megaLayers, tab.data(), tab.size() * sizeof(dl::MegaLayer), cudaMemcpyHostToDevice));
         DL_CUDA_CHECK(cudaMalloc(&e->megaCounter, 256));
         DL_CUDA_CHECK(cudaMemset(e->megaCounter, 0, 256));
-        const dl::EngineConfig &c = e->cfg;
         const size_t qDim = (size_t)c.nHeads * c.headDim, qkvDim = qDim + 2 * (size_t)c.nKvHeads * c.headDim;
         auto allocW = [](uint2 **p, size_t n) {
             const size_t bytes = (n + 8) * sizeof(uint2);
@@ -498,9 +518,6 @@
             std::memset(e->abortHost, 0, 64);
             DL_CUDA_CHECK(cudaHostGetDevicePointer((void **)&e->abortDev, e->abortHost, 0));
         }
-        if (const char *g = std::getenv("DL_MEGA_CTAS")) e->megaCtas = (uint32_t)std::atoi(g);
-        if (const char *g = std::getenv("DL_MEGA_FLAGS")) e->megaFlags = (uint32_t)std::atoi(g);
-        if (const char *g = std::getenv("DL_MEGA_INFLIGHT")) e->megaInflight = (uint32_t)std::atoi(g);
     }
     e->useMega = enable != 0;
     return 0;
diff --git a/csrc/cuda/kernels.h b/csrc/cuda/kernels.h
--- a/csrc/cuda/kernels.h
+++ b/csrc/cuda/kernels.h
@@ -145,6 +145,7 @@
 
 struct MegaLayer {
     const uint8_t *qkvQs, *qkvSc, *woQs, *woSc, *w13Qs, *w13Sc, *w2Qs, *w2Sc;
+    const uint8_t *w2bQs, *w2bSc;
     const float *norm0, *norm1, *qNorm, *kNorm;
     __nv_bfloat16 *kCache, *vCache;
 };
@@ -169,6 +170,10 @@
     uint32_t flags;
     uint2 *xW, *qkvW, *zW;
     float *hF;
+    uint2 *hW;
+    uint2 *ffPartW;
+    uint32_t ffK, ffSlabRows;
+    uint32_t ffLeftQ, ffLeftRem;
     unsigned int *launchSeq;
     unsigned int *abortFlag;
     unsigned long long *syncNs;
@@ -190,6 +195,7 @@
 };
 
 int launchMegaDecode(MegaArgs m, int numSms, cudaStream_t stream);
+int launchBlockMajorQ40(const void *qs, const void *scales, uint32_t rows, uint32_t nb, void *dstQs, void *dstScales, cudaStream_t stream);
 
 enum { GEPI_STORE_F32_ = 0, GEPI_RESIDUAL_ = 1, GEPI_SWIGLU_BF16_ = 2, GEPI_STORE_BF16_ = 3 };
 int gemmQ40Tc(int epi, const void *qs, const void *scales, uint32_t d, uint32_t n, const void *act, uint32_t actStride, uint32_t T,
diff --git a/csrc/cuda/mega_decode.cu b/csrc/cuda/mega_decode.cu
--- a/csrc/cuda/mega_decode.cu
+++ b/csrc/cuda/mega_decode.cu
@@ -111,94 +111,50 @@
     tileRows = 2 * (P.pairsQ + (b < P.pairsRem ? 1u : 0u));
 }
 
-template <int PRO, int EPI, bool IN_PLAIN = false>
-__device__ void megaGemv(const MegaArgs &m, const MegaSmem &sm, const MegaPhase &P, const uint2 *in, uint32_t inEpoch, const float *normW,
-                         uint2 *outW, uint32_t outEpoch, float *outF, uint32_t arParity, RingPos &ring, int tid, uint32_t &slot,
-                         const float *inF = nullptr, const uint2 *resW = nullptr) {
-    auto stamp = [&]() { if (m.trace && tid == 0 && blockIdx.x < m.traceCtas) m.trace[(size_t)blockIdx.x * m.traceStride + slot] = globalTimerNs(); slot++; };
+__device__ __forceinline__ void q80Put(float4 v, uint32_t i, bool act, uint8_t *pa, uint8_t *pb, float *dxs, float *dx8) {
+    float amax = fmaxf(fmaxf(fabsf(v.x), fabsf(v.y)), fmaxf(fabsf(v.z), fabsf(v.w)));
+    amax = fmaxf(amax, __shfl_xor_sync(0xffffffffu, amax, 1));
+    amax = fmaxf(amax, __shfl_xor_sync(0xffffffffu, amax, 2));
+    amax = fmaxf(amax, __shfl_xor_sync(0xffffffffu, amax, 4));
+    const float dq = amax / 127.f;
+    const float id = dq != 0.f ? 1.f / dq : 0.f;
+    const int q0 = __float2int_rn(v.x * id), q1 = __float2int_rn(v.y * id);
+    const int q2 = __float2int_rn(v.z * id), q3 = __float2int_rn(v.w * id);
+    int qsum = q0 + q1 + q2 + q3;
+    qsum += __shfl_xor_sync(0xffffffffu, qsum, 1);
+    qsum += __shfl_xor_sync(0xffffffffu, qsum, 2);
+    qsum += __shfl_xor_sync(0xffffffffu, qsum, 4);
+    if (act) {
+        const uint32_t b = i >> 3, sub = i & 7, kk = sub >> 1, odd = sub & 1;
+        uint8_t *wa = pa + (size_t)b * 16 + kk * 4 + odd;
+        uint8_t *wb = pb + (size_t)b * 16 + kk * 4 + odd;
+        wa[0] = (uint8_t)(int8_t)q0; wa[2] = (uint8_t)(int8_t)q1;
+        wb[0] = (uint8_t)(int8_t)q2; wb[2] = (uint8_t)(int8_t)q3;
+        if (sub == 0) {
+            const float dr = __half2float(__float2half_rn(dq));
+            dxs[b] = dr;
+            dx8[b] = dr * 8.f * (float)qsum;
+        }
+    }
+}
+
+__device__ __forceinline__ float q40Dot(const uint4 q, float dw, const uint4 A, const uint4 B, float dxv, float dx8v) {
+    const uint32_t ml = 0x0f0f0f0fu, mh = 0xf0f0f0f0u;
+    int lo = dp4a(q.x & ml, A.x, 0), hi = dp4a(q.x & mh, B.x, 0);
+    lo = dp4a(q.y & ml, A.y, lo); hi = dp4a(q.y & mh, B.y, hi);
+    lo = dp4a(q.z & ml, A.z, lo); hi = dp4a(q.z & mh, B.z, hi);
+    lo = dp4a(q.w & ml, A.w, lo); hi = dp4a(q.w & mh, B.w, hi);
+    return dw * (dxv * (float)(lo + (hi >> 4)) - dx8v);
+}
+
+__device__ __forceinline__ void megaMainLoop(const MegaArgs &m, const MegaSmem &sm, const MegaPhase &P, uint32_t tileRows, RingPos &ring, int tid) {
     const int lane = tid & 31, warp = tid >> 5;
-    const uint32_t n = P.n;
     const uint32_t nblk = P.nblk, nseg = P.nseg;
     const uint32_t rowQsBytes = nblk * 16;
-    uint32_t pairBegin, tileRows;
-    megaTile(P, pairBegin, tileRows);
-    const uint32_t rowBase = pairBegin * 2;
     const uint32_t SR = P.stageRows;
-    uint4 *planeA = sm.planeA, *planeB = sm.planeB;
-    float *dxs = sm.dxs, *dx8 = sm.dx8, *partial = sm.partial, *red = sm.red;
-
-    float resid = 0.f;
-    if (EPI == EPI_RESIDUAL_ && (uint32_t)tid < tileRows) resid = __uint_as_float(ldW((resW ? resW : outW) + rowBase + tid).x);
-
-    {
-        const uint32_t nVec = n / 4;
-        constexpr int kMaxVec = PRO == PRO_RMSNORM_ ? 4 : 8;
-        constexpr uint32_t kChunkVec = kMaxVec * kConsumerThreads;
-        uint8_t *pa = reinterpret_cast<uint8_t *>(planeA);
-        uint8_t *pb = reinterpret_cast<uint8_t *>(planeB);
-        for (uint32_t vecBase = 0; vecBase < nVec; vecBase += kChunkVec) {
-            float4 xv[kMaxVec];
-            float4 wv[PRO == PRO_RMSNORM_ ? kMaxVec : 1];
-            if (PRO == PRO_RMSNORM_) {
-#pragma unroll
-                for (int k = 0; k < kMaxVec; k++) {
-                    const uint32_t i = vecBase + k * kConsumerThreads + tid;
-                    wv[k] = i < nVec ? __ldg(reinterpret_cast<const float4 *>(normW) + i) : make_float4(0.f, 0.f, 0.f, 0.f);
-                }
-            }
-            float ss = 0.f;
-#pragma unroll
-            for (int k = 0; k < kMaxVec; k++) {
-                const uint32_t i = vecBase + k * kConsumerThreads + tid;
-                if (IN_PLAIN) xv[k] = i < nVec ? __ldcg(reinterpret_cast<const float4 *>(inF) + i) : make_float4(0.f, 0.f, 0.f, 0.f);
-                else xv[k] = i < nVec ? ldW4wait(in, i, inEpoch, m.abortFlag) : make_float4(0.f, 0.f, 0.f, 0.f);
-                ss += xv[k].x * xv[k].x + xv[k].y * xv[k].y + xv[k].z * xv[k].z + xv[k].w * xv[k].w;
-            }
-            float inv = 1.f;
-            if (PRO == PRO_RMSNORM_) {
-                ss = consumerSum(ss, red);
-                inv = rsqrtf(ss / (float)n + m.eps);
-            }
-#pragma unroll
-            for (int k = 0; k < kMaxVec; k++) {
-                const uint32_t i = vecBase + k * kConsumerThreads + tid;
-                if (vecBase + k * kConsumerThreads >= nVec) break;
-                const bool act = i < nVec;
-                float4 v = xv[k];
-                if (PRO == PRO_RMSNORM_ && act) {
-                    const float4 w = wv[PRO == PRO_RMSNORM_ ? k : 0];
-                    v.x = w.x * (v.x * inv); v.y = w.y * (v.y * inv); v.z = w.z * (v.z * inv); v.w = w.w * (v.w * inv);
-                }
-                float amax = fmaxf(fmaxf(fabsf(v.x), fabsf(v.y)), fmaxf(fabsf(v.z), fabsf(v.w)));
-                amax = fmaxf(amax, __shfl_xor_sync(0xffffffffu, amax, 1));
-                amax = fmaxf(amax, __shfl_xor_sync(0xffffffffu, amax, 2));
-                amax = fmaxf(amax, __shfl_xor_sync(0xffffffffu, amax, 4));
-                const float dq = amax / 127.f;
-                const float id = dq != 0.f ? 1.f / dq : 0.f;
-                const int q0 = __float2int_rn(v.x * id), q1 = __float2int_rn(v.y * id);
-                const int q2 = __float2int_rn(v.z * id), q3 = __float2int_rn(v.w * id);
-                int qsum = q0 + q1 + q2 + q3;
-                qsum += __shfl_xor_sync(0xffffffffu, qsum, 1);
-                qsum += __shfl_xor_sync(0xffffffffu, qsum, 2);
-                qsum += __shfl_xor_sync(0xffffffffu, qsum, 4);
-                if (act) {
-                    const uint32_t b = i >> 3, sub = i & 7, kk = sub >> 1, odd = sub & 1;
-                    uint8_t *wa = pa + (size_t)b * 16 + kk * 4 + odd;
-                    uint8_t *wb = pb + (size_t)b * 16 + kk * 4 + odd;
-                    wa[0] = (uint8_t)(int8_t)q0; wa[2] = (uint8_t)(int8_t)q1;
-                    wb[0] = (uint8_t)(int8_t)q2; wb[2] = (uint8_t)(int8_t)q3;
-                    if (sub == 0) {
-                        const float dr = __half2float(__float2half_rn(dq));
-                        dxs[b] = dr;
-                        dx8[b] = dr * 8.f * (float)qsum;
-                    }
-                }
-            }
-        }
-    }
-    consumerBarrier();
-    stamp();
-
+    const uint4 *planeA = sm.planeA, *planeB = sm.planeB;
+    const float *dxs = sm.dxs, *dx8 = sm.dx8;
+    float *partial = sm.partial;
     const uint32_t gInc = P.gInc, segInc = P.segInc;
     uint32_t rot = 0;
     for (uint32_t r0 = 0; r0 < tileRows; r0 += SR) {
@@ -226,12 +182,7 @@
                 for (int r = 0; r < kRowsPerStep; r++) {
                     const uint4 q = qp[r * nblk];
                     const float dw = __half2float(__ushort_as_half(sp[r * nblk]));
-                    const uint32_t ml = 0x0f0f0f0fu, mh = 0xf0f0f0f0u;
-                    int lo = dp4a(q.x & ml, A.x, 0), hi = dp4a(q.x & mh, B.x, 0);
-                    lo = dp4a(q.y & ml, A.y, lo); hi = dp4a(q.y & mh, B.y, hi);
-                    lo = dp4a(q.z & ml, A.z, lo); hi = dp4a(q.z & mh, B.z, hi);
-                    lo = dp4a(q.w & ml, A.w, lo); hi = dp4a(q.w & mh, B.w, hi);
-                    acc[r] = dw * (dxv * (float)(lo + (hi >> 4)) - dx8v);
+                    acc[r] = q40Dot(q, dw, A, B, dxv, dx8v);
                 }
             }
         };
@@ -271,13 +222,84 @@
         ring.advance(m.nStages);
     }
     consumerBarrier();
+}
+
+__device__ __forceinline__ float megaRowSum(const MegaSmem &sm, uint32_t nseg, uint32_t r) {
+    float v = 0.f;
+    for (uint32_t sg = 0; sg < nseg; sg++) v += sm.partial[r * nseg + sg];
+    return v;
+}
+
+template <int PRO, bool IN_PLAIN>
+__device__ __forceinline__ void megaPrologue(const MegaArgs &m, const MegaSmem &sm, uint32_t n, const uint2 *in, uint32_t inEpoch,
+                                             const float *normW, const float *inF, int tid) {
+    const uint32_t nVec = n / 4;
+    constexpr int kMaxVec = PRO == PRO_RMSNORM_ ? 4 : 8;
+    constexpr uint32_t kChunkVec = kMaxVec * kConsumerThreads;
+    uint8_t *pa = reinterpret_cast<uint8_t *>(sm.planeA);
+    uint8_t *pb = reinterpret_cast<uint8_t *>(sm.planeB);
+    for (uint32_t vecBase = 0; vecBase < nVec; vecBase += kChunkVec) {
+        float4 xv[kMaxVec];
+        float4 wv[PRO == PRO_RMSNORM_ ? kMaxVec : 1];
+        if (PRO == PRO_RMSNORM_) {
+#pragma unroll
+            for (int k = 0; k < kMaxVec; k++) {
+                const uint32_t i = vecBase + k * kConsumerThreads + tid;
+                wv[k] = i < nVec ? __ldg(reinterpret_cast<const float4 *>(normW) + i) : make_float4(0.f, 0.f, 0.f, 0.f);
+            }
+        }
+        float ss = 0.f;
+#pragma unroll
+        for (int k = 0; k < kMaxVec; k++) {
+            const uint32_t i = vecBase + k * kConsumerThreads + tid;
+            if (IN_PLAIN) xv[k] = i < nVec ? __ldcg(reinterpret_cast<const float4 *>(inF) + i) : make_float4(0.f, 0.f, 0.f, 0.f);
+            else xv[k] = i < nVec ? ldW4wait(in, i, inEpoch, m.abortFlag) : make_float4(0.f, 0.f, 0.f, 0.f);
+            ss += xv[k].x * xv[k].x + xv[k].y * xv[k].y + xv[k].z * xv[k].z + xv[k].w * xv[k].w;
+        }
+        float inv = 1.f;
+        if (PRO == PRO_RMSNORM_) {
+            ss = consumerSum(ss, sm.red);
+            inv = rsqrtf(ss / (float)n + m.eps);
+        }
+#pragma unroll
+        for (int k = 0; k < kMaxVec; k++) {
+            const uint32_t i = vecBase + k * kConsumerThreads + tid;
+            if (vecBase + k * kConsumerThreads >= nVec) break;
+            const bool act = i < nVec;
+            float4 v = xv[k];
+            if (PRO == PRO_RMSNORM_ && act) {
+                const float4 w = wv[PRO == PRO_RMSNORM_ ? k : 0];
+                v.x = w.x * (v.x * inv); v.y = w.y * (v.y * inv); v.z = w.z * (v.z * inv); v.w = w.w * (v.w * inv);
+            }
+            q80Put(v, i, act, pa, pb, sm.dxs, sm.dx8);
+        }
+    }
+    consumerBarrier();
+}
+
+template <int PRO, int EPI, bool IN_PLAIN = false>
+__device__ void megaGemv(const MegaArgs &m, const MegaSmem &sm, const MegaPhase &P, const uint2 *in, uint32_t inEpoch, const float *normW,
+                         uint2 *outW, uint32_t outEpoch, float *outF, uint32_t arParity, RingPos &ring, int tid, uint32_t &slot,
+                         const float *inF = nullptr, const uint2 *resW = nullptr) {
+    auto stamp = [&]() { if (m.trace && tid == 0 && blockIdx.x < m.traceCtas) m.trace[(size_t)blockIdx.x * m.traceStride + slot] = globalTimerNs(); slot++; };
+    const int lane = tid & 31, warp = tid >> 5;
+    const uint32_t n = P.n;
+    const uint32_t nseg = P.nseg;
+    uint32_t pairBegin, tileRows;
+    megaTile(P, pairBegin, tileRows);
+    const uint32_t rowBase = pairBegin * 2;
+    float *red = sm.red;
+
+    float resid = 0.f;
+    if (EPI == EPI_RESIDUAL_ && (uint32_t)tid < tileRows) resid = __uint_as_float(ldW((resW ? resW : outW) + rowBase + tid).x);
+
+    megaPrologue<PRO, IN_PLAIN>(m, sm, n, in, inEpoch, normW, inF, tid);
     stamp();
 
-    auto rowSum = [&](uint32_t r) {
-        float v = 0.f;
-        for (uint32_t sg = 0; sg < nseg; sg++) v += partial[r * nseg + sg];
-        return v;
-    };
+    megaMainLoop(m, sm, P, tileRows, ring, tid);
+    stamp();
+
+    auto rowSum = [&](uint32_t r) { return megaRowSum(sm, nseg, r); };
     if (EPI == EPI_SWIGLU_) {
         for (uint32_t p = tid; p < tileRows / 2; p += kConsumerThreads) outF[pairBegin + p] = gateAct(rowSum(2 * p), m.act) * rowSum(2 * p + 1);
     } else if (EPI == EPI_STORE_) {
@@ -400,6 +422,127 @@
                 }
             }
         }
+    }
+}
+
+__device__ void megaFfnFused(const MegaArgs &m, const MegaSmem &sm, const MegaLayer &L, const uint2 *xIn, uint32_t inEpoch, uint2 *xOut,
+                             uint32_t outEpoch, RingPos &ring, int tid, uint32_t &slot, unsigned int *ctr, unsigned int &barTarget) {
+    auto stamp = [&]() { if (m.trace && tid == 0 && blockIdx.x < m.traceCtas) m.trace[(size_t)blockIdx.x * m.traceStride + slot] = globalTimerNs(); slot++; };
+    const int lane = tid & 31, warp = tid >> 5;
+    const MegaPhase &P = m.ph[MP_W13];
+    const uint32_t nseg = P.nseg, dim = m.dim, c = blockIdx.x, G = gridDim.x, k = m.ffK;
+    const uint32_t left0 = k * G, nLeft = m.ffDim / 32 - left0;
+    const uint32_t hEpoch = inEpoch + 1;
+    uint8_t *pa = reinterpret_cast<uint8_t *>(sm.planeA), *pb = reinterpret_cast<uint8_t *>(sm.planeB);
+
+    megaPrologue<PRO_RMSNORM_, false>(m, sm, dim, xIn, inEpoch, L.norm1, nullptr, tid);
+    stamp();
+
+    const uint32_t lpBegin = c * m.ffLeftQ + min(c, m.ffLeftRem), lpRows = 2 * (m.ffLeftQ + (c < m.ffLeftRem ? 1u : 0u));
+    if (lpRows) {
+        megaMainLoop(m, sm, P, lpRows, ring, tid);
+        for (uint32_t p = tid; p < lpRows / 2; p += kConsumerThreads)
+            stW(m.hW + left0 * 32 + lpBegin + p, gateAct(megaRowSum(sm, nseg, 2 * p), m.act) * megaRowSum(sm, nseg, 2 * p + 1), hEpoch);
+        consumerBarrier();
+    }
+    megaMainLoop(m, sm, P, 64 * k, ring, tid);
+    stamp();
+
+    for (uint32_t vb = 0; vb < 8 * k; vb += kConsumerThreads) {
+        const uint32_t i = vb + tid;
+        const bool act = i < 8 * k;
+        float4 v = make_float4(0.f, 0.f, 0.f, 0.f);
+        if (act) {
+            const uint32_t e = 4 * i;
+            v.x = gateAct(megaRowSum(sm, nseg, 2 * e), m.act) * megaRowSum(sm, nseg, 2 * e + 1);
+            v.y = gateAct(megaRowSum(sm, nseg, 2 * e + 2), m.act) * megaRowSum(sm, nseg, 2 * e + 3);
+            v.z = gateAct(megaRowSum(sm, nseg, 2 * e + 4), m.act) * megaRowSum(sm, nseg, 2 * e + 5);
+            v.w = gateAct(megaRowSum(sm, nseg, 2 * e + 6), m.act) * megaRowSum(sm, nseg, 2 * e + 7);
+        }
+        q80Put(v, i, act, pa, pb, sm.dxs, sm.dx8);
+    }
+    for (uint32_t vb = 0; vb < 8 * nLeft; vb += kConsumerThreads) {
+        const uint32_t i = vb + tid;
+        const bool act = i < 8 * nLeft;
+        const float4 v = act ? ldW4wait(m.hW + left0 * 32, i, hEpoch, m.abortFlag) : make_float4(0.f, 0.f, 0.f, 0.f);
+        q80Put(v, i, act, pa + k * 16, pb + k * 16, sm.dxs + k, sm.dx8 + k);
+    }
+    consumerBarrier();
+    uint32_t pairBegin, tileRows;
+    megaTile(m.ph[MP_W2], pairBegin, tileRows);
+    const uint32_t rowBase = 2 * pairBegin;
+    float *red = sm.partial, *lsum = sm.partial + kConsumerThreads;
+    if (nLeft) {
+        const uint4 *bq = reinterpret_cast<const uint4 *>(L.w2bQs) + (size_t)left0 * dim + rowBase;
+        const __half *bs = reinterpret_cast<const __half *>(L.w2bSc) + (size_t)left0 * dim + rowBase;
+        for (uint32_t r = warp; r < tileRows; r += kConsumerWarps) {
+            float s = 0.f;
+            for (uint32_t j = lane; j < nLeft; j += 32)
+                s += q40Dot(__ldg(bq + (size_t)j * dim + r), __half2float(bs[(size_t)j * dim + r]), sm.planeA[k + j], sm.planeB[k + j],
+                            sm.dxs[k + j], sm.dx8[k + j]);
+            s = warpSum(s);
+            if (lane == 0) lsum[r] = s;
+        }
+    } else {
+        for (uint32_t r = tid; r < tileRows; r += kConsumerThreads) lsum[r] = 0.f;
+    }
+    stamp();
+
+    {
+        const uint32_t SR = m.ffSlabRows;
+        uint2 *part = m.ffPartW + (size_t)c * dim;
+        for (uint32_t r0 = 0; r0 < dim; r0 += SR) {
+            const uint32_t st = ring.st;
+            const uint32_t rows = min(SR, dim - r0);
+            const uint8_t *stage = sm.ring + st * m.stageBytes;
+            const uint4 *sq = reinterpret_cast<const uint4 *>(stage);
+            const uint16_t *ss = reinterpret_cast<const uint16_t *>(stage + (size_t)k * SR * 16);
+            mbarWait(&sm.fullBar[st], ring.par);
+            for (uint32_t r = tid; r < rows; r += kConsumerThreads) {
+                float acc = 0.f;
+                for (uint32_t j = 0; j < k; j++)
+                    acc += q40Dot(sq[j * SR + r], __half2float(__ushort_as_half(ss[j * SR + r])), sm.planeA[j], sm.planeB[j], sm.dxs[j], sm.dx8[j]);
+                stW(part + r0 + r, acc, hEpoch);
+            }
+            __syncwarp();
+            if (lane == 0) mbarArrive(&sm.emptyBar[st]);
+            ring.advance(m.nStages);
+        }
+    }
+    stamp();
+
+    if (m.flags & 2u) gridBarrier(ctr, barTarget, tid, m.abortFlag);
+    for (uint32_t rb = 0; rb < tileRows; rb += 32) {
+        const uint32_t r = rb + lane;
+        const float resid = (warp == 0 && r < tileRows) ? __uint_as_float(ldW(xIn + rowBase + r).x) : 0.f;
+        float s = 0.f;
+        if (r < tileRows) {
+            const uint2 *src = m.ffPartW + rowBase + r;
+            constexpr uint32_t kBatch = 10;
+            for (uint32_t c0 = warp; c0 < G; c0 += kBatch * kConsumerWarps) {
+                uint2 w[kBatch];
+#pragma unroll
+                for (uint32_t u = 0; u < kBatch; u++) {
+                    const uint32_t cc = c0 + u * kConsumerWarps;
+                    w[u] = cc < G ? ldW(src + (size_t)cc * dim) : make_uint2(0u, hEpoch);
+                }
+#pragma unroll
+                for (uint32_t u = 0; u < kBatch; u++) {
+                    const uint32_t cc = c0 + u * kConsumerWarps;
+                    if (w[u].y != hEpoch) w[u].x = __float_as_uint(ldWwait(src + (size_t)cc * dim, hEpoch, m.abortFlag));
+                    s += __uint_as_float(w[u].x);
+                }
+            }
+        }
+        red[warp * 32 + lane] = s;
+        consumerBarrier();
+        if (warp == 0 && r < tileRows) {
+            float v = 0.f;
+#pragma unroll
+            for (int w = 0; w < kConsumerWarps; w++) v += red[w * 32 + lane];
+            stW(xOut + rowBase + r, resid + (v + lsum[r]), outEpoch);
+        }
+        consumerBarrier();
     }
 }
 
@@ -654,36 +797,70 @@
             RingPos landed{0u, 0u};
             uint32_t nIssued = 0, nLanded = 0;
             const uint32_t maxInflight = m.maxInflight ? m.maxInflight : m.nStages;
-            auto stream = [&](const uint8_t *qs, const uint8_t *sc, const MegaPhase &P) {
+            auto acquire = [&]() {
+                const uint32_t st = pr.st;
+                if (wrapped) mbarWait(&sm.emptyBar[st], pr.par ^ 1u);
+                while (nIssued - nLanded >= maxInflight) {
+                    mbarWait(&sm.fullBar[landed.st], landed.par);
+                    landed.advance(m.nStages);
+                    nLanded++;
+                }
+                nIssued++;
+                return st;
+            };
+            auto release = [&]() {
+                pr.advance(m.nStages);
+                if (pr.st == 0) wrapped = true;
+            };
+            auto streamRows = [&](const uint8_t *qs, const uint8_t *sc, const MegaPhase &P, uint32_t rowBase, uint32_t tileRows) {
                 const uint32_t rowQsBytes = P.nblk * 16, rowScBytes = P.nblk * 2;
-                uint32_t pairBegin, tileRows;
-                megaTile(P, pairBegin, tileRows);
-                const uint32_t rowBase = pairBegin * 2, SR = P.stageRows;
+                const uint32_t SR = P.stageRows;
                 for (uint32_t r0 = 0; r0 < tileRows; r0 += SR) {
-                    const uint32_t st = pr.st;
-                    if (wrapped) mbarWait(&sm.emptyBar[st], pr.par ^ 1u);
-                    while (nIssued - nLanded >= maxInflight) {
-                        mbarWait(&sm.fullBar[landed.st], landed.par);
-                        landed.advance(m.nStages);
-                        nLanded++;
-                    }
-                    nIssued++;
+                    const uint32_t st = acquire();
                     const uint32_t rows = min(SR, tileRows - r0);
                     const uint32_t bq = rows * rowQsBytes, bs = rows * rowScBytes;
                     uint8_t *dst = sm.ring + st * m.stageBytes;
                     mbarExpectTx(&sm.fullBar[st], bq + bs);
                     tmaBulkLoad(dst, qs + (uint64_t)(rowBase + r0) * rowQsBytes, bq, &sm.fullBar[st], policy);
                     tmaBulkLoad(dst + SR * rowQsBytes, sc + (uint64_t)(rowBase + r0) * rowScBytes, bs, &sm.fullBar[st], policy);
-                    pr.advance(m.nStages);
-                    if (pr.st == 0) wrapped = true;
+                    release();
                 }
             };
+            auto stream = [&](const uint8_t *qs, const uint8_t *sc, const MegaPhase &P) {
+                uint32_t pairBegin, tileRows;
+                megaTile(P, pairBegin, tileRows);
+                streamRows(qs, sc, P, pairBegin * 2, tileRows);
+            };
+            auto streamSlab = [&](const uint8_t *qs, const uint8_t *sc) {
+                const uint32_t k = m.ffK, SR = m.ffSlabRows, blk0 = blockIdx.x * k;
+                for (uint32_t r0 = 0; r0 < m.dim; r0 += SR) {
+                    const uint32_t st = acquire();
+                    const uint32_t rows = min(SR, m.dim - r0);
+                    uint8_t *dst = sm.ring + st * m.stageBytes;
+                    mbarExpectTx(&sm.fullBar[st], rows * k * 18);
+                    for (uint32_t j = 0; j < k; j++) {
+                        const uint64_t at = (uint64_t)(blk0 + j) * m.dim + r0;
+                        tmaBulkLoad(dst + j * SR * 16, qs + at * 16, rows * 16, &sm.fullBar[st], policy);
+                        tmaBulkLoad(dst + k * SR * 16 + j * SR * 2, sc + at * 2, rows * 2, &sm.fullBar[st], policy);
+                    }
+                    release();
+                }
+            };
+            const uint32_t c = blockIdx.x;
+            const uint32_t lpRows = 2 * (m.ffLeftQ + (c < m.ffLeftRem ? 1u : 0u));
+            const uint32_t lpRowBase = 2 * (m.ffK * gridDim.x * 32 + c * m.ffLeftQ + min(c, m.ffLeftRem));
             for (uint32_t l = 0; l < m.nLayers; l++) {
                 const MegaLayer &L = m.layers[l];
                 stream(L.qkvQs, L.qkvSc, m.ph[MP_QKV]);
                 stream(L.woQs, L.woSc, m.ph[MP_WO]);
-                stream(L.w13Qs, L.w13Sc, m.ph[MP_W13]);
-                stream(L.w2Qs, L.w2Sc, m.ph[MP_W2]);
+                if (m.ffK) {
+                    streamRows(L.w13Qs, L.w13Sc, m.ph[MP_W13], lpRowBase, lpRows);
+                    streamRows(L.w13Qs, L.w13Sc, m.ph[MP_W13], c * m.ffK * 64, m.ffK * 64);
+                    streamSlab(L.w2bQs, L.w2bSc);
+                } else {
+                    stream(L.w13Qs, L.w13Sc, m.ph[MP_W13]);
+                    stream(L.w2Qs, L.w2Sc, m.ph[MP_W2]);
+                }
             }
             stream(m.wclsQs, m.wclsSc, m.ph[MP_LOGITS]);
         }
@@ -733,11 +910,15 @@
         stamp();
         llBarrier();
         stamp();
-        megaGemv<PRO_RMSNORM_, EPI_SWIGLU_>(m, sm, m.ph[MP_W13], xB, e0 + 3, L.norm1, nullptr, 0, m.hF, 0, ring, tid, slot);
-        stamp();
-        gridBarrierFenced(m.gridCounter, barTarget, tid, m.abortFlag);
-        stamp();
-        megaGemv<PRO_PLAIN_, EPI_RESIDUAL_, true>(m, sm, m.ph[MP_W2], nullptr, 0, nullptr, xA, e0 + 5, nullptr, 1, ring, tid, slot, m.hF, xB);
+        if (m.ffK) {
+            megaFfnFused(m, sm, L, xB, e0 + 3, xA, e0 + 5, ring, tid, slot, m.gridCounter, barTarget);
+        } else {
+            megaGemv<PRO_RMSNORM_, EPI_SWIGLU_>(m, sm, m.ph[MP_W13], xB, e0 + 3, L.norm1, nullptr, 0, m.hF, 0, ring, tid, slot);
+            stamp();
+            gridBarrierFenced(m.gridCounter, barTarget, tid, m.abortFlag);
+            stamp();
+            megaGemv<PRO_PLAIN_, EPI_RESIDUAL_, true>(m, sm, m.ph[MP_W2], nullptr, 0, nullptr, xA, e0 + 5, nullptr, 1, ring, tid, slot, m.hF, xB);
+        }
         stamp();
         llBarrier();
     }
@@ -770,6 +951,9 @@
         const uint32_t nseg = (dn[i] / 32 + 31) / 32;
         if (tile * nseg > partial) partial = tile * nseg;
     }
+    const uint32_t nbH = m.ffDim / 32;
+    const bool ffFused = m.ffPartW && nbH >= grid && m.ar.nRanks <= 1 && !(m.flags & 1u);
+    if (ffFused && kConsumerThreads + 2 * (m.dim / 2 / grid + 1) > partial) partial = kConsumerThreads + 2 * (m.dim / 2 / grid + 1);
     m.partialFloats = (partial + 3) / 4 * 4;
     m.planeBlocks = maxN / 32;
     const size_t fixedBytes = (size_t)m.planeBlocks * (16 + 16 + 4 + 4) + (size_t)m.partialFloats * 4 + 32 * 4 + 128 * 4 + 2 * kMaxStages * 8 + 256;
@@ -798,6 +982,20 @@
             if (((sft * P.recipNseg) >> 16) != sft / P.nseg) return 1;
     }
     if (2 * (m.ph[MP_WO].pairsQ + 1) > (uint32_t)kConsumerThreads) return 1;
+    m.ffK = 0;
+    if (ffFused) {
+        const uint32_t k = nbH / grid, rowBytes = k * 18;
+        uint32_t sr = stageBytes / (rowBytes * kConsumerThreads) * kConsumerThreads;
+        if (sr == 0) sr = stageBytes / rowBytes / 32 * 32;
+        if (sr > m.dim) sr = m.dim;
+        if (sr >= 32) {
+            const uint32_t leftPairs = (nbH - k * grid) * 32;
+            m.ffK = k;
+            m.ffSlabRows = sr;
+            m.ffLeftQ = leftPairs / grid;
+            m.ffLeftRem = leftPairs % grid;
+        }
+    }
     const size_t smemBytes = fixedBytes + (size_t)stages * stageBytes;
     const int v = m.headDim == 128 ? 1 : 0;
     int dev = 0;
diff --git a/csrc/cuda/repack.cu b/csrc/cuda/repack.cu
--- a/csrc/cuda/repack.cu
+++ b/csrc/cuda/repack.cu
@@ -69,6 +69,25 @@
     }
 }
 
+__global__ void __launch_bounds__(256) blockMajorQ40Kernel(const uint4 *qs, const __half *scales, uint32_t rows, uint32_t nb, uint4 *dstQs,
+                                                          __half *dstScales) {
+    const uint64_t total = (uint64_t)rows * nb;
+    for (uint64_t i = (uint64_t)blockIdx.x * blockDim.x + threadIdx.x; i < total; i += (uint64_t)gridDim.x * blockDim.x) {
+        const uint32_t b = (uint32_t)(i / rows), r = (uint32_t)(i % rows);
+        dstQs[i] = qs[(uint64_t)r * nb + b];
+        dstScales[i] = scales[(uint64_t)r * nb + b];
+    }
+}
+
+int launchBlockMajorQ40(const void *qs, const void *scales, uint32_t rows, uint32_t nb, void *dstQs, void *dstScales, cudaStream_t stream) {
+    const uint64_t total = (uint64_t)rows * nb;
+    if (total == 0) return 0;
+    const int grid = (int)((total + 255) / 256 < 148 * 16 ? (total + 255) / 256 : 148 * 16);
+    blockMajorQ40Kernel<<<grid, 256, 0, stream>>>((const uint4 *)qs, (const __half *)scales, rows, nb, (uint4 *)dstQs, (__half *)dstScales);
+    DL_CUDA_CHECK(cudaGetLastError());
+    return 0;
+}
+
 }
 
 DL_EXPORT int dl_repack_q40(const void *src, uint64_t srcRowPitch, uint64_t srcColByteOffset, uint32_t rows,
```

Measured after the change: 720.1 tokens/s, median of 6. 0.87x the previous value.
